# osudrl/cassie-mujoco-sim

Hardware: AMD Instinct MI355X
Metric: env-steps/sec (whole node) at N envs; max |qpos_err| vs CPU ref (higher is better)
Workload: dtype f64

## Files before the change

cassie-mujoco-sim_amd/csrc/env_step_collision.inc:

```
        constexpr int chain_rounds = [] {
            if constexpr (TOPO::is_static) { int r = 0, n = 1; while (n < DofLevels<TOPO>::depth() + 1) { n *= 4; ++r; } return r < 3 ? r : 3; }
            else return 3;
        }();
        int pf_jlim, pf_jtype, pf_jqadr, danc[9], blast, kvin;
        double pf_jmargin, pf_jlo, pf_jhi;
        auto request_behind_collision = [&](int lane_now) {
            const int pf_lj = lane_now < njnt ? lane_now : 0, pf_kd = lane_now < nv ? lane_now : 0, pf_bb = lane_now < nbody ? lane_now : 0;
            pf_jlim = m->jnt_limited[pf_lj]; pf_jtype = m->jnt_type[pf_lj]; pf_jqadr = m->jnt_qposadr[pf_lj];
            pf_jmargin = m->jnt_margin[pf_lj]; pf_jlo = m->jnt_range[pf_lj][0]; pf_jhi = m->jnt_range[pf_lj][1];
#pragma unroll
            for (int r = 0; r < 3 * chain_rounds; ++r) danc[r] = m->dof_anc4[pf_kd][r];
            blast = m->body_lastdof[pf_bb]; kvin = m->dof_vinsrc[pf_kd];
        };
        constexpr bool request_early = (FEAT & FEAT_HFIELD) == 0;
        if constexpr (request_early) request_behind_collision(lane);
        const int pair_bound = m->npair_simple;
        struct PairConst { int g1, g2, tt; double margin, rb1, rb2, s10, s11, s20, s21, s22; };
        auto request_pair = [&](int pp, PairConst &c) {
            const int ps = pp < pair_bound ? pp : 0;
            c.g1 = m->pair_geom1[ps]; c.g2 = m->pair_geom2[ps]; c.tt = m->pair_type[ps];
            c.margin = m->pair_margin[ps]; c.rb1 = m->pair_rbound[ps][0]; c.rb2 = m->pair_rbound[ps][1];
            c.s10 = m->pair_size[ps][0]; c.s11 = m->pair_size[ps][1];
            c.s20 = m->pair_size[ps][3]; c.s21 = m->pair_size[ps][4]; c.s22 = m->pair_size[ps][5];
        };
        PairConst pc;
        if constexpr (request_early) request_pair(lane, pc);
        int ncon = 0;
        int npass = m->npair_always;
        if (m->npair_simple > m->npair_always) {
            bool nearby = false;
            if (lane < m->ngeom && m->geom_farstatic[lane]) {
                const double rb = m->geom_rbound[lane] + m->geom_margin[lane];
                for (int ri = 0; ri < m->nroot; ++ri) {
                    const int r = m->root_body[ri];
                    double dv[3] = {S.x.s.geom_xpos[lane][0] - S.x.s.xpos[r][0], S.x.s.geom_xpos[lane][1] - S.x.s.xpos[r][1],
                                    S.x.s.geom_xpos[lane][2] - S.x.s.xpos[r][2]};
                    const double bound = PG->body_reach[r] + rb + 0.01;
                    if (dot3(dv, dv) < bound * bound) nearby = true;
                }
            }
            if (wv::ballot(nearby) != 0ull) npass = m->npair_simple;
        }
        CK_STAMP(21);
        constexpr int HF_REC = 1 + 10 * CM_HF_MAXC;
        static_assert(CM_MAXHFPAIR * HF_REC <= NB * 12 + NVP * 12, "the height-field result table must fit the cvel + cfrc + cdof_dot + buf tiles");
        static_assert(offsetof(decltype(S.x.s), buf) - offsetof(decltype(S.x.s), cvel) == sizeof(double) * (NB * 12 + NVP * 6), "those four tiles are contiguous");
        static_assert(CM_HF_PASS * CM_HF_SLOTS <= WV_WAVE && CM_HF_SLOTS_DENSE <= WV_WAVE, "a pass of the height-field pre-pass is one wave");
        double *const hfres = &S.x.s.cvel[0][0];
        const bool hf_on = (FEAT & FEAT_HFIELD) != 0 && env_hfield != nullptr && m->nhfpair > 0;
        const bool hf_prism = (FEAT & FEAT_HFIELD) != 0 && hf_on && (m->flags & CM_FLAG_HFPRISM) != 0;
        int ncon_prism = 0;
        if constexpr ((FEAT & FEAT_HFIELD) != 0) if (hf_prism) {
            static_assert(CM_MAXHFPAIR * HP_REC + 64 * 2 * CM_HP_MAXS / 8 <= NB * 12 + NVP * 12, "the per-pair records of the prism pass and its task table (a byte per task) fit the idle velocity tiles");
            CK_STAMP(44);
            ncon_prism = hfield_prism_wave(S, m, env_hfield, lane, hfres, MAXC);
            CK_STAMP(46);
        }
        if constexpr ((FEAT & FEAT_HFIELD) != 0) if (hf_on && !hf_prism) {
            const bool dense = (m->flags & CM_FLAG_HFDENSE) != 0;
            const int slots = dense ? CM_HF_SLOTS_DENSE : CM_HF_SLOTS, per_pass = dense ? WV_WAVE / CM_HF_SLOTS_DENSE : CM_HF_PASS;
            for (int h0 = 0; h0 < m->nhfpair; h0 += per_pass) {
                const int hl = dense ? lane / CM_HF_SLOTS_DENSE : lane / CM_HF_SLOTS;
                const int h = h0 + hl, k = lane - hl * slots;
                const bool act = hl < per_pass && h < m->nhfpair;
                const int p = m->hfpair[act ? h : 0];
                const int g1 = m->pair_geom1[p], g2 = m->pair_geom2[p], t2 = m->pair_type[p] >> 8;
                const double margin = m->pair_margin[p], s20 = m->pair_size[p][3], s21 = m->pair_size[p][4];
                const double *p1 = S.x.s.geom_xpos[g1], *m1 = S.x.s.geom_xmat[g1], *p2 = S.x.s.geom_xpos[g2], *m2 = S.x.s.geom_xmat[g2];
                const double axis[3] = {m2[2], m2[5], m2[8]};
                const double cell = 2 * m->hfield_size[0] / (m->hfield_ncol > 1 ? m->hfield_ncol - 1 : 1);
                int ni = 0;
                bool mine = act && k == 0;
                double t = 0;
                if (t2 == CM_GEOM_CAPSULE) {
                    ni = (int)ceil(2 * s21 / cell) - 1;
                    if (ni < 0) ni = 0;
                    if (ni > slots - 2) ni = slots - 2;
                    mine = act && k < 2 + ni;
                    t = k == 0 ? s21 : (k == 1 ? -s21 : s21 * (1.0 - 2.0 * (k - 1) / (ni + 1)));
                }
                RawContact rcs;
                rcs.dist = 1e300;
                bool has = false;
                {
                    double e[3] = {p2[0] + t * axis[0], p2[1] + t * axis[1], p2[2] + t * axis[2]};
                    static_assert(offsetof(SH_T, c_tran) + sizeof(S.c_tran) - offsetof(SH_T, c_dist) >= (size_t)HF_WORK_BYTES,
                                  "the contact tables hold the work area of hfield_spheres_wave");
                    CK_STAMP(44);
                    has = hfield_spheres_wave(rcs, m, env_hfield, p1, m1, mine, e, s20, margin, lane, &S.c_dist[0]) != 0;
                    CK_STAMP(45);
                }
                const int lead = lane - k;
                double dk[CM_HF_SLOTS_DENSE];
                const double mydist = has ? rcs.dist : 1e300;
#pragma unroll
                for (int q = 0; q < CM_HF_SLOTS_DENSE; ++q) {
                    if (q >= CM_HF_SLOTS && !dense) { dk[q] = 1e300; continue; }
                    const double v = wv::shfl(mydist, (lead + q) & 63);
                    dk[q] = q < slots ? v : 1e300;
                }
                int src0 = 0, src1 = 1;
                bool have0 = dk[0] < 1e299, have1 = dk[1] < 1e299;
                if (t2 == CM_GEOM_CAPSULE) {
                    int kmid = -1;
                    double dmid = 1e300;
#pragma unroll
                    for (int q = 2; q < CM_HF_SLOTS_DENSE; ++q) if (dk[q] < 1e299 && (kmid < 0 || dk[q] < dmid)) { kmid = q; dmid = dk[q]; }
                    if (kmid >= 0 && (!have0 || dmid < dk[0]) && (!have1 || dmid < dk[1])) {
                        const bool drop1 = !have0 ? false : (!have1 ? true : dk[0] <= dk[1]);
                        if (drop1) { src1 = kmid; have1 = true; } else { src0 = kmid; have0 = true; }
                    }
                } else {
                    have1 = false;
                }
                int nkeep = (have0 ? 1 : 0) + (have1 ? 1 : 0);
                double *rec = hfres + (size_t)(act ? h : 0) * HF_REC;
                int slot_of_me = (have0 && k == src0) ? 0 : ((have1 && k == src1) ? (have0 ? 1 : 0) : -1);
                if ((m->flags & CM_FLAG_HFMULTI) && t2 == CM_GEOM_CAPSULE) {
                    int rank = 0, cnt = 0;
#pragma unroll
                    for (int q = 0; q < CM_HF_SLOTS_DENSE; ++q) {
                        const bool valid = dk[q] < 1e299;
                        cnt += valid ? 1 : 0;
                        rank += (valid && (dk[q] < mydist || (dk[q] == mydist && q < k))) ? 1 : 0;
                    }
                    nkeep = cnt < CM_HF_MAXC ? cnt : CM_HF_MAXC;
                    slot_of_me = (has && rank < CM_HF_MAXC) ? rank : -1;
                }
                if (act && k == 0) rec[0] = (double)nkeep;
                if (act && slot_of_me >= 0) {
                    double *c = rec + 1 + 10 * slot_of_me;
                    c[0] = rcs.dist;
                    for (int i = 0; i < 3; ++i) { c[1 + i] = rcs.pos[i]; c[4 + i] = rcs.normal[i]; c[7 + i] = t2 == CM_GEOM_CAPSULE ? axis[i] : 0.0; }
                }
            }
            wv::sync();
            CK_STAMP(46);
        }
        if constexpr (!request_early) request_pair(lane, pc);
        if constexpr ((FEAT & FEAT_HFIELD) != 0) ncon = ncon_prism;
        for (int p0 = 0; p0 < npass; p0 += WV_WAVE) {
            const int p = p0 + lane;
            int n = 0;
            RawContact rc0, rc1;
            bool from_spread = false;
            int hfs = -1;
            if constexpr ((FEAT & FEAT_HFIELD) != 0) {
                const int slot = p < npass ? m->pair_hfslot[p] : -1;
                if (slot >= 0) {
                    from_spread = true;
                    if (hf_on && !hf_prism) {
                        const double *rec = hfres + (size_t)slot * HF_REC;
                        n = (int)rec[0];
                        hfs = slot;
                        rc0.dist = rec[1]; rc1.dist = rec[11];
                        for (int i = 0; i < 3; ++i) {
                            rc0.pos[i] = rec[2 + i]; rc0.normal[i] = rec[5 + i]; rc0.tangent[i] = rec[8 + i];
                            rc1.pos[i] = rec[12 + i]; rc1.normal[i] = rec[15 + i]; rc1.tangent[i] = rec[18 + i];
                        }
                    }
                }
            }
            if (p < npass && !from_spread) {
                const int g1 = pc.g1, g2 = pc.g2, tt = pc.tt;
                const int t1 = tt & 255, t2 = tt >> 8;
                const double margin = pc.margin;
                const double *p1 = S.x.s.geom_xpos[g1], *p2 = S.x.s.geom_xpos[g2];
                const double *m1 = S.x.s.geom_xmat[g1], *m2 = S.x.s.geom_xmat[g2];
                const double rb1 = pc.rb1, rb2 = pc.rb2;
                const double s10 = pc.s10, s11 = pc.s11, s20 = pc.s20, s21 = pc.s21, s22 = pc.s22;
                double dif[3] = {p2[0] - p1[0], p2[1] - p1[1], p2[2] - p1[2]};
                CK_STAMP(31);
                bool cull = false;
                if (rb1 > 0 && rb2 > 0) {
                    double bound = rb1 + rb2 + margin;
                    cull = dot3(dif, dif) > bound * bound;
                } else if (t1 == CM_GEOM_PLANE && rb2 > 0) {
                    double nn[3] = {m1[2], m1[5], m1[8]};
                    cull = dot3(dif, nn) > margin + rb2;
                }
                if (!cull) {
                    if (t1 == CM_GEOM_PLANE && t2 == CM_GEOM_SPHERE) {
                        n = plane_sphere(rc0, p1, m1, p2, s20, margin);
                    } else if (t1 == CM_GEOM_PLANE && t2 == CM_GEOM_CAPSULE) {
                        double axis[3] = {m2[2], m2[5], m2[8]};
                        RawContact tmp;
                        double e0[3] = {p2[0] + s21 * axis[0], p2[1] + s21 * axis[1], p2[2] + s21 * axis[2]};
                        if (plane_sphere(tmp, p1, m1, e0, s20, margin)) { rc0 = tmp; n = 1; }
                        double e1[3] = {p2[0] - s21 * axis[0], p2[1] - s21 * axis[1], p2[2] - s21 * axis[2]};
                        if (plane_sphere(tmp, p1, m1, e1, s20, margin)) { if (n == 0) rc0 = tmp; else rc1 = tmp; ++n; }
                        for (int i = 0; i < 3; ++i) { rc0.tangent[i] = axis[i]; rc1.tangent[i] = axis[i]; }
                    } else if (t1 == CM_GEOM_SPHERE && t2 == CM_GEOM_SPHERE) {
                        n = sphere_sphere(rc0, p1, s10, p2, s20, margin);
                    } else if (t1 == CM_GEOM_SPHERE && t2 == CM_GEOM_CAPSULE) {
                        double a2[3] = {m2[2], m2[5], m2[8]};
                        double d12[3] = {-dif[0], -dif[1], -dif[2]};
                        double x = clampd(dot3(a2, d12), -s21, s21);
                        double q2[3] = {p2[0] + a2[0] * x, p2[1] + a2[1] * x, p2[2] + a2[2] * x};
                        n = sphere_sphere(rc0, p1, s10, q2, s20, margin);
                    } else if (t1 == CM_GEOM_CAPSULE && t2 == CM_GEOM_CAPSULE) {
                        double a1[3] = {m1[2], m1[5], m1[8]}, a2[3] = {m2[2], m2[5], m2[8]};
                        double x1, x2;
                        segment_closest(p1, a1, s11, p2, a2, s21, x1, x2);
                        double q1[3] = {p1[0] + a1[0] * x1, p1[1] + a1[1] * x1, p1[2] + a1[2] * x1};
                        double q2[3] = {p2[0] + a2[0] * x2, p2[1] + a2[1] * x2, p2[2] + a2[2] * x2};
                        n = sphere_sphere(rc0, q1, s10, q2, s20, margin);
                    } else if (t1 == CM_GEOM_SPHERE && t2 == CM_GEOM_BOX) {
                        double sb[3] = {s20, s21, s22};
                        n = sphere_box(rc0, p1, s10, p2, m2, sb, margin);
                    } else if (t1 == CM_GEOM_CAPSULE && t2 == CM_GEOM_BOX) {
                        double sb[3] = {s20, s21, s22};
                        n = capsule_box(rc0, rc1, p1, m1, s10, s11, p2, m2, sb, margin);
                    } else {
                        warn |= WARN_UNSUPPORTED_PAIR;
                    }
                }
            }
            CK_STAMP(32);
            if (p0 + WV_WAVE < npass) request_pair(p + WV_WAVE, pc);
            const unsigned long long m1b = wv::ballot(n >= 1), m2b = wv::ballot(n >= 2);
            const unsigned long long below = (lane == 0) ? 0ull : (~0ull >> (64 - lane));
            int slot = ncon + wv::popc64(m1b & below) + wv::popc64(m2b & below);
            int more = 0;
            if constexpr ((FEAT & FEAT_HFIELD) != 0) {
                const unsigned long long m3b = wv::ballot(n >= 3), m4b = wv::ballot(n >= 4);
                slot += wv::popc64(m3b & below) + wv::popc64(m4b & below);
                more = wv::popc64(m3b) + wv::popc64(m4b);
                for (int extra = 2; extra < CM_HF_MAXC; ++extra)
                    if (n > extra && slot + extra < MAXC) {
                        const double *c = hfres + (size_t)hfs * HF_REC + 1 + 10 * extra;
                        RawContact rx;
                        rx.dist = c[0];
                        for (int i = 0; i < 3; ++i) { rx.pos[i] = c[1 + i]; rx.normal[i] = c[4 + i]; rx.tangent[i] = c[7 + i]; }
                        write_raw_contact(S, slot + extra, p, rx);
                    }
            }
            if (n >= 1 && slot < MAXC) write_raw_contact(S, slot, p, rc0);
            if (n >= 2 && slot + 1 < MAXC) write_raw_contact(S, slot + 1, p, rc1);
            ncon += wv::popc64(m1b) + wv::popc64(m2b) + more;
        }
        CK_STAMP(22);
        if constexpr (!request_early) request_behind_collision(lane);
        if constexpr ((FEAT & FEAT_WAVEPAIRS) != 0) for (int p = m->npair_simple; p < m->npair; ++p) {
            const int g1 = m->pair_geom1[p], g2 = m->pair_geom2[p], tt = m->pair_type[p];
            const int t1 = tt & 255, t2 = tt >> 8;
            const double margin = m->pair_margin[p];
            const double *p1 = S.x.s.geom_xpos[g1], *p2 = S.x.s.geom_xpos[g2];
            const double *m1 = S.x.s.geom_xmat[g1], *m2 = S.x.s.geom_xmat[g2];
            const double rb1 = m->pair_rbound[p][0], rb2 = m->pair_rbound[p][1];
            {
                double dif[3] = {p2[0] - p1[0], p2[1] - p1[1], p2[2] - p1[2]};
                bool cull = false;
                if (rb1 > 0 && rb2 > 0) { const double bound = rb1 + rb2 + margin; cull = dot3(dif, dif) > bound * bound; }
                else if (t1 == CM_GEOM_PLANE && rb2 > 0) { double nn[3] = {m1[2], m1[5], m1[8]}; cull = dot3(dif, nn) > margin + rb2; }
                if (cull) continue;
            }
            bool hit = false;
            int pairmax = 4;
            RawContact rc;
            if (t1 == CM_GEOM_PLANE && t2 == CM_GEOM_BOX) {
                if (lane < 8) {
                    const double sb0 = m->pair_size[p][3], sb1 = m->pair_size[p][4], sb2 = m->pair_size[p][5];
                    double nrm[3] = {m1[2], m1[5], m1[8]}, dif[3] = {p2[0] - p1[0], p2[1] - p1[1], p2[2] - p1[2]};
                    const double dist = dot3(dif, nrm);
                    double v[3] = {(lane & 1) ? sb0 : -sb0, (lane & 2) ? sb1 : -sb1, (lane & 4) ? sb2 : -sb2}, corner[3];
                    mulmatvec3(corner, m2, v);
                    const double ld = dot3(nrm, corner);
                    if (!(dist + ld > margin || ld > 0)) {
                        hit = true;
                        rc.dist = dist + ld;
                        for (int k = 0; k < 3; ++k) { rc.normal[k] = nrm[k]; rc.tangent[k] = 0; rc.pos[k] = corner[k] + p2[k] - nrm[k] * 0.5 * rc.dist; }
                    }
                }
            } else if (t1 == CM_GEOM_BOX && t2 == CM_GEOM_BOX) {
                double s1[3] = {m->pair_size[p][0], m->pair_size[p][1], m->pair_size[p][2]};
                double s2[3] = {m->pair_size[p][3], m->pair_size[p][4], m->pair_size[p][5]};
                pairmax = (m->flags & CM_FLAG_BOX8) ? 8 : 4;
                hit = box_box_lane(rc, lane, p1, m1, s1, p2, m2, s2, margin, pairmax);
            } else {
                warn |= WARN_UNSUPPORTED_PAIR;
            }
            const unsigned long long hb = wv::ballot(hit);
            const unsigned long long below = (lane == 0) ? 0ull : (~0ull >> (64 - lane));
            const int rank = wv::popc64(hb & below);
            if (hit && rank < pairmax && ncon + rank < MAXC) write_raw_contact(S, ncon + rank, p, rc);
            const int nh = wv::popc64(hb);
            ncon += nh < pairmax ? nh : pairmax;
        }
        const int ncon_found = ncon;
        if (ncon > capc) ncon = capc;
        wv::sync();
        finish_contacts(S, m, P, lane, ncon);
        unsigned long long lob, hib;
        {
            bool lo = false, hi = false;
            wv::keep(pf_jlim); wv::keep(pf_jtype);
            if (lane < njnt && pf_jlim && (pf_jtype == CM_JNT_HINGE || pf_jtype == CM_JNT_SLIDE)) {
                const double q = S.qpos[pf_jqadr];
                lo = q - pf_jlo < pf_jmargin;
                hi = pf_jhi - q < pf_jmargin;
            }
            lob = wv::ballot(lo); hib = wv::ballot(hi);
        }
        if constexpr (MAXR < WIDE_ROWS) {
            const bool may_go_down = io.down_rows > 0 && sub > sub_start;
            if (can_hand_over || may_go_down) {
                const int neq = m->neq;
                const bool eact = lane < neq && m->eq_active[lane < neq ? lane : 0] != 0;
                wv::sync();
                const int nfrictionless = wv::popc64(wv::ballot(lane < ncon && S.c_dim[lane < MAXC ? lane : 0] == 1));
                const int need = 3 * wv::popc64(wv::ballot(eact)) + wv::popc64(lob) + wv::popc64(hib) + 4 * ncon - 3 * nfrictionless;
                const bool up = can_hand_over && (need > capr || (ncon_found > capc && MAXC < m->maxcon));
                const bool down = !up && may_go_down && need <= io.down_rows;
                if (up || down) {
                    bailed = true; bailed_down = down;
                    if constexpr (NW == 2) { if (lane == 0) S.cmd[0] = 1; wv::publish(&S.cmd[4], sub + 1); }
                    break;
                }
            }
        }
        if (ncon_found > capc) warn |= WARN_CONTACT_FULL;
        if constexpr (NW == 1) if (io.drive_mode) {
            if (io.integrate) drive_level_io(io, S, m, env, lane, lastsub);
            wv::sync();
        }
        if constexpr (NW == 2) { CK_STAMP(33); wv::publish(&S.cmd[4], sub + 1); wv::wait_for(&S.cmd[3], sub + 1); }
        CK_STAMP(5);
```

cassie-mujoco-sim_amd/csrc/env_step_rows.inc:

```
        int r_ = lane;
        int rtype = -1, rid = 0, rsub = 0;
        int nefc = 0, nefc_before_contacts = 0;
        double rpos = 0, rmargin = 0, rR = 1.0, rK = 0, rB = 0, rimp = 1.0;
        const bool need_imu = lastsub || io.all_outputs_every_substep || (io.drive_mode && sub + 2 == nsub);
        const bool need_pos = lastsub || io.drive_mode || io.all_outputs_every_substep;
        const bool issens = lane < m->nsensor && need_pos;
        const int ls = issens ? lane : 0;
        SensorConsts sens_c;
        double ycol[NVP];
        double jvel = 0, jws = 0;
        const bool lastcol = !WIDE && lane == NROW - 1;
        for (int pass = 0; pass < (WIDE ? 2 : 1); ++pass) {
        if constexpr (WIDE) {
            if (pass == 1 && nefc <= NROW) break;
            r_ = NROW * pass + lane; rtype = -1; rid = 0; rsub = 0; nefc = 0; jvel = 0; jws = 0;
            rpos = 0; rmargin = 0; rR = 1.0; rK = 0; rB = 0; rimp = 1.0;
        }
        {
            const int neq = m->neq;
            const bool eact = lane < neq && m->eq_active[lane < neq ? lane : 0] != 0;
            const unsigned long long eall = neq >= 64 ? ~0ull : (1ull << neq) - 1;
            if (wv::ballot(eact) == eall && 3 * neq <= capr) {
                if (r_ < 3 * neq) { rtype = CM_CNSTR_EQUALITY; rid = r_ / 3; rsub = r_ - 3 * rid; }
                nefc = 3 * neq;
            } else
            for (int e = 0; e < neq; ++e) {
                if (!m->eq_active[e]) continue;
                if (nefc + 3 > capr) { warn |= WARN_CONSTRAINT_FULL; continue; }
                if (r_ >= nefc && r_ < nefc + 3) { rtype = CM_CNSTR_EQUALITY; rid = e; rsub = r_ - nefc; }
                nefc += 3;
            }
        }
        {
            for (unsigned long long any = lob | hib; any; any &= any - 1) {
                const int j = wv::popc64((any & (0ull - any)) - 1);
                for (int side = 0; side < 2; ++side) {
                    if (!(((side == 0 ? lob : hib) >> j) & 1ull)) continue;
                    if (nefc >= capr) { warn |= WARN_CONSTRAINT_FULL; continue; }
                    if (r_ == nefc) { rtype = CM_CNSTR_LIMIT_JOINT; rid = j; rsub = side; }
                    ++nefc;
                }
            }
        }
        nefc_before_contacts = nefc;
        const bool cpyr = lane < ncon && S.c_dim[lane < ncon ? lane : 0] == 3;
        if (wv::ballot(cpyr) == (ncon >= 64 ? ~0ull : (1ull << ncon) - 1) && nefc + 4 * ncon <= capr) {
            if (r_ >= nefc && r_ < nefc + 4 * ncon) { rtype = CM_CNSTR_CONTACT_PYRAMIDAL; rid = (r_ - nefc) >> 2; rsub = (r_ - nefc) & 3; }
            nefc += 4 * ncon;
        } else
        for (int c = 0; c < ncon; ++c) {
            const int dim = S.c_dim[c];
            if (dim != 1 && dim != 3) { warn |= WARN_UNSUPPORTED_PAIR; continue; }
            const int nrow = dim == 1 ? 1 : 2 * (dim - 1);
            if (nefc + nrow > capr) { warn |= WARN_CONSTRAINT_FULL; continue; }
            if (r_ >= nefc && r_ < nefc + nrow) {
                rtype = dim == 1 ? CM_CNSTR_CONTACT_FRICTIONLESS : CM_CNSTR_CONTACT_PYRAMIDAL;
                rid = c; rsub = r_ - nefc;
            }
            nefc += nrow;
        }

        CK_STAMP(25);
        double u3[3] = {0, 0, 0}, wp[3] = {0, 0, 0}, wm[3] = {0, 0, 0};
        unsigned long long maskp = 0, maskm = 0;
        int limdof = -1;
        double limsgn = 0, rdiag = 0, imp_pos = 0, rRscale = 1.0;
        double solref0 = 0.02, solref1 = 1, solimp[5] = {0.9, 0.95, 0.001, 0.5, 2};
        if (rtype == CM_CNSTR_EQUALITY) {
            if (rid != pf_eq) {
                pf_eb1 = m->eq_body1[rid]; pf_eb2 = m->eq_body2[rid]; pf_er1 = m->eq_root[rid][0]; pf_er2 = m->eq_root[rid][1];
            }
            maskp = m->eq_dofmask[rid][0]; maskm = m->eq_dofmask[rid][1];
            rdiag = P->eq_invweight[rid];
            solref0 = m->eq_solref[rid][0]; solref1 = m->eq_solref[rid][1];
            for (int i = 0; i < 5; ++i) solimp[i] = m->eq_solimp[rid][i];
            const int b1 = pf_eb1, b2 = pf_eb2;
            double l1[3] = {m->eq_data[rid][0], m->eq_data[rid][1], m->eq_data[rid][2]};
            double l2[3] = {m->eq_data[rid][3], m->eq_data[rid][4], m->eq_data[rid][5]};
            double a1[3], a2[3];
            mulmatvec3(a1, S.x.s.xmat[b1], l1);
            mulmatvec3(a2, S.x.s.xmat[b2], l2);
            for (int i = 0; i < 3; ++i) { a1[i] += S.x.s.xpos[b1][i]; a2[i] += S.x.s.xpos[b2][i]; }
            u3[0] = rsub == 0 ? 1.0 : 0.0; u3[1] = rsub == 1 ? 1.0 : 0.0; u3[2] = rsub == 2 ? 1.0 : 0.0;
            const double *c1 = S.com[pf_er1], *c2 = S.com[pf_er2];
            double o1[3] = {a1[0] - c1[0], a1[1] - c1[1], a1[2] - c1[2]};
            double o2[3] = {a2[0] - c2[0], a2[1] - c2[1], a2[2] - c2[2]};
            cross3(wp, o1, u3);
            cross3(wm, o2, u3);

            double res[3] = {a1[0] - a2[0], a1[1] - a2[1], a1[2] - a2[2]};
            rpos = rsub == 0 ? res[0] : (rsub == 1 ? res[1] : res[2]); rmargin = 0;
            imp_pos = sqrt(dot3(res, res));

        } else if (rtype == CM_CNSTR_LIMIT_JOINT) {
            const double q = S.qpos[m->jnt_qposadr[rid]];
            rpos = rsub == 0 ? q - m->jnt_range[rid][0] : m->jnt_range[rid][1] - q;
            rmargin = m->jnt_margin[rid];
            imp_pos = rpos;
            limdof = m->jnt_dofadr[rid];
            limsgn = rsub == 0 ? 1.0 : -1.0;
            rdiag = P->jnt_liminvweight[rid];
            solref0 = m->jnt_solref[rid][0]; solref1 = m->jnt_solref[rid][1];
            for (int i = 0; i < 5; ++i) solimp[i] = m->jnt_solimp[rid][i];
        } else if (rtype >= 0) {
            const int c = rid;
            const double *fr = S.c_frame[c];
            if (rtype == CM_CNSTR_CONTACT_PYRAMIDAL) {
                const int a = 1 + rsub / 2;
                const double mu = a <= 2 ? S.c_fri[c][0] : (a == 3 ? S.c_fri[c][1] : S.c_fri[c][2]);
                const double sg = (rsub & 1) ? -mu : mu;
                for (int i = 0; i < 3; ++i) u3[i] = fr[i] + sg * fr[3 * a + i];
                const double mu0 = S.c_fri[c][0];
                rRscale = 2 * mu0 * mu0;
            } else {
                for (int i = 0; i < 3; ++i) u3[i] = fr[i];
            }
            const double *c1 = S.com[S.c_root[c][0]], *c2 = S.com[S.c_root[c][1]];
            double o1[3] = {S.c_pos[c][0] - c1[0], S.c_pos[c][1] - c1[1], S.c_pos[c][2] - c1[2]};
            double o2[3] = {S.c_pos[c][0] - c2[0], S.c_pos[c][1] - c2[1], S.c_pos[c][2] - c2[2]};
            cross3(wp, o2, u3);
            cross3(wm, o1, u3);
            maskp = S.c_dofmask[c][1];
            maskm = S.c_dofmask[c][0];
            rpos = S.c_dist[c]; rmargin = S.c_margin[c]; imp_pos = rpos;
            const double tran = S.c_tran[c];
            const double mu_first = S.c_fri[c][0];
            rdiag = rtype == CM_CNSTR_CONTACT_PYRAMIDAL ? tran + mu_first * mu_first * tran : tran;
            solref0 = S.c_solref[c][0]; solref1 = S.c_solref[c][1];
            for (int i = 0; i < 5; ++i) solimp[i] = S.c_solimp[c][i];
        }
        CK_STAMP(26);
        if (rtype >= 0) {
            rimp = impedance(solimp, imp_pos, rmargin);
            rR = fmax(CM_MINVAL, (1 - rimp) * rdiag / rimp);
            if (rtype == CM_CNSTR_CONTACT_PYRAMIDAL) rR = fmax(CM_MINVAL, rRscale * rR);
            const double dmax = solimp[1];
            if (solref0 > 0) {
                double tc = solref0;
                if ((m->flags & CM_FLAG_REFSAFE) && tc < 2 * h) tc = 2 * h;
                rK = 1.0 / fmax(CM_MINVAL, dmax * dmax * tc * tc * solref1 * solref1);
                rB = 2.0 / fmax(CM_MINVAL, dmax * tc);
            } else {
                rK = -solref0 / fmax(CM_MINVAL, dmax * dmax);
                rB = -solref1 / fmax(CM_MINVAL, dmax);
            }
        }
        CK_STAMP(27);
        if constexpr (NW == 1) sens_c = request_sensor_consts(m, ls);
#pragma unroll
        for (int k0 = 0; k0 < NVP; k0 += 4) {
            double cc[4][6], qv[4], qw[4], qs[4];
#pragma unroll
            for (int kk = 0; kk < 4; ++kk) {
#pragma unroll
                for (int t = 0; t < 6; ++t) cc[kk][t] = S.cdof[k0 + kk][t];
                qv[kk] = S.qvel[k0 + kk]; qw[kk] = S.qacc_ws[k0 + kk];
                if constexpr (NW == 1) qs[kk] = S.qfrc_smooth[k0 + kk]; else qs[kk] = 0.0;
            }
            wv::sched_fence();
#pragma unroll
            for (int kk = 0; kk < 4; ++kk) {
                const int k = k0 + kk;
                double v = 0;
                if (TOPO::is_static ? k < TOPO::nv : k < nv) {
                    if (rtype >= 0) {
                        const double ul = u3[0] * cc[kk][3] + u3[1] * cc[kk][4] + u3[2] * cc[kk][5];
                        const double sp = bitf(maskp, k), sm = bitf(maskm, k);
                        v = sp * (ul + wp[0] * cc[kk][0] + wp[1] * cc[kk][1] + wp[2] * cc[kk][2]) -
                            sm * (ul + wm[0] * cc[kk][0] + wm[1] * cc[kk][1] + wm[2] * cc[kk][2]);
                        if (k == limdof) v = limsgn;
                        jvel += v * qv[kk];
                        jws += v * qw[kk];
                    } else if (lastcol) {
                        v = qs[kk];
                    }
                }
                ycol[k] = v;
            }
        }
        if constexpr (WIDE) {
            if (r_ < MAXR) {
#pragma unroll
                for (int k = 0; k < NVP; ++k) S.x.Yr[r_][k] = ycol[k];
                double *rt = S.x.rowt[r_];
                rt[0] = rR; rt[1] = rtype >= 0 ? -rB * jvel - rK * rimp * (rpos - rmargin) : 0.0; rt[2] = jws;
                rt[3] = rtype < 0 ? -1.0 : (rtype == CM_CNSTR_EQUALITY ? 0.0 : 1.0);
            }
            if (io.ext && pass == 0 && rtype == CM_CNSTR_EQUALITY && r_ < CM_MAXEQROW) {
                cm_ext_t *ex = io.ext + env;
                ex->eq_pos[r_] = rpos; ex->eq_id[r_] = rid;
#pragma unroll
                for (int k = 0; k < NVP; ++k) if (k < nv) ex->eq_J[r_][k] = ycol[k];
            }
        }
        }
        const int sb = NW == 1 ? sens_c.sb : 0;
        CK_STAMP(28);
        if constexpr (NW == 2) {
            if constexpr (WIDE) { if (lane == 0) S.x.turn[0] = nefc; }
            CK_STAMP(34); wv::block_barrier();
            if (lastcol) {
#pragma unroll
                for (int k = 0; k < NVP; ++k) ycol[k] = (TOPO::is_static ? k < TOPO::nv : k < nv) ? S.qfrc_smooth[k] : 0.0;
            }
        }
        const double raref = rtype >= 0 ? -rB * jvel - rK * rimp * (rpos - rmargin) : 0.0;

        int aslot = -1;
        if constexpr (NW == 1) aslot = sensors_before_solve(io, S, m, env, issens, ls, sens_c, need_imu, lastsub);
        CK_STAMP(29);
        if (io.xpos_out && isbody && lastsub) {
            for (int i = 0; i < 3; ++i) io.xpos_out[((size_t)env * io.sb + b) * 3 + i] = S.x.s.xpos[b][i];
            if (io.xquat_out) for (int i = 0; i < 4; ++i) io.xquat_out[((size_t)env * io.sb + b) * 4 + i] = S.x.s.xquat[b][i];
        }
        if (io.ext) {
            cm_ext_t *ex = io.ext + env;
            if (isbody) for (int i = 0; i < 6; ++i) ex->cvel[b][i] = S.x.s.cvel[b][i];
            if (isbody) for (int i = 0; i < 3; ++i) { ex->subtree_com[b][i] = S.com[broot > 0 ? broot : 0][i]; ex->xipos[b][i] = S.x.s.xipos[b][i]; }
            if (lane < m->nsite) {
                const int sb = m->site_bodyid[lane];
                double sp[3] = {m->site_pos[lane][0], m->site_pos[lane][1], m->site_pos[lane][2]};
                double sq[4] = {m->site_quat[lane][0], m->site_quat[lane][1], m->site_quat[lane][2], m->site_quat[lane][3]};
                double t[3], q[4], mm[9];
                mulmatvec3(t, S.x.s.xmat[sb], sp);
                for (int i = 0; i < 3; ++i) ex->site_xpos[lane][i] = t[i] + S.x.s.xpos[sb][i];
                mulquat(q, S.x.s.xquat[sb], sq);
                quat2mat(mm, q);
                for (int i = 0; i < 9; ++i) ex->site_xmat[lane][i] = mm[i];
            }
            if (isdof) for (int i = 0; i < 6; ++i) { ex->cdof[k_][i] = S.cdof[k_][i]; ex->cdof_dot[k_][i] = S.x.s.cdof_dot[k_][i]; }
            if (!WIDE && rtype == CM_CNSTR_EQUALITY && r_ < CM_MAXEQROW) {
                ex->eq_pos[r_] = rpos; ex->eq_id[r_] = rid;
#pragma unroll
                for (int k = 0; k < NVP; ++k) if (k < nv) ex->eq_J[r_][k] = ycol[k];
            }
            if (lane == 0) { int ne = 0; for (int e = 0; e < m->neq; ++e) if (m->eq_active[e] && ne + 3 <= capr) ne += 3; ex->ne = ne; }
            if (lane < ncon) {
                ex->con_geom1[lane] = m->geom_fullid[S.c_g1[lane]]; ex->con_geom2[lane] = m->geom_fullid[S.c_g2[lane]];
                ex->con_body1[lane] = m->geom_bodyid[S.c_g1[lane]]; ex->con_body2[lane] = m->geom_bodyid[S.c_g2[lane]];
                ex->con_dim[lane] = S.c_dim[lane]; ex->con_dist[lane] = S.c_dist[lane];
                for (int i = 0; i < 3; ++i) ex->con_pos[lane][i] = S.c_pos[lane][i];
                for (int i = 0; i < 9; ++i) ex->con_frame[lane][i] = S.c_frame[lane][i];
            }
        }
        int caddr = -1;
        const bool want_cfrc = io.body_cfrc && (sub == nsub - 1 || !io.integrate);
        if (io.ext || want_cfrc) {
            int acc = nefc_before_contacts;
            for (int c = 0; c < ncon; ++c) {
                const int dim = S.c_dim[c];
                if (dim != 1 && dim != 3) continue;
                const int nrow = dim == 1 ? 1 : 2 * (dim - 1);
                if (acc + nrow > capr) continue;
                if (c == lane) caddr = acc;
                acc += nrow;
            }
        }
        wv::sync();
        CK_STAMP(8);
```

cassie-mujoco-sim_amd/csrc/env_step_solve.inc:

```
        if constexpr (WIDE) {
            int iters = 0, nguarded = 0;
            const double f = wide_solve<NVP, TOPO>(S, m, P, 0, nefc, sub, iters, nguarded);
            CK_STAMP(11);

            static_assert(sizeof(S.c_solimp) >= (2 * NROW + 4) * sizeof(double), "the row forces are handed over through the contacts' solimp slots");
            double *const fbuf = &S.c_solimp[0][0];
            fbuf[lane] = f;
            if (lane == 0) { fbuf[2 * NROW] = (double)ncon; fbuf[2 * NROW + 1] = (double)nefc; fbuf[2 * NROW + 2] = (double)iters; fbuf[2 * NROW + 3] = (double)nguarded; }
            wv::block_barrier();
#ifdef CK_WIDE_PROFILE
            if (io.prof && lane < 12) io.prof[(size_t)env * NSTAMP + (lane < 6 ? 16 + lane : 22 + lane)] = (long long)S.x.stepv[lane / 6][lane % 6];
#endif
            if (io.ext || want_cfrc) {
                const int a0 = caddr >= 0 ? caddr : 0;
                double fn = 0, ft1 = 0, ft2 = 0;
                if (lane < ncon && caddr >= 0) {
                    const double f0 = fbuf[a0];
                    if (S.c_dim[lane] == 1) fn = f0;
                    else { const double f1 = fbuf[a0 + 1], f2 = fbuf[a0 + 2], f3 = fbuf[a0 + 3], mu = S.c_fri[lane][0]; fn = f0 + f1 + f2 + f3; ft1 = mu * (f0 - f1); ft2 = mu * (f2 - f3); }
                }
                if (io.ext) {
                    cm_ext_t *ex = io.ext + env;
                    if (lane < ncon) { ex->con_force[lane][0] = fn; ex->con_force[lane][1] = ft1; ex->con_force[lane][2] = ft2; }
                    if (lane == 0) { ex->ncon = ncon; ex->nefc = nefc; ex->solver_iter = iters; }
                }
                if (want_cfrc) {
                    if (lane < ncon) {
                        const double *fr = S.c_frame[lane];
                        double fw[3];
                        for (int j = 0; j < 3; ++j) fw[j] = fr[j] * fn + fr[3 + j] * ft1 + fr[6 + j] * ft2;
                        for (int j = 0; j < 3; ++j) S.c_pos[lane][j] = fw[j];
                    }
                    wv::sync();
                    if (isbody) {
                        double acc[3] = {0, 0, 0};
                        for (int c = 0; c < ncon; ++c) {
                            const int b1 = m->geom_bodyid[S.c_g1[c]], b2 = m->geom_bodyid[S.c_g2[c]];
                            const double sg = (b2 == b ? 1.0 : 0.0) - (b1 == b ? 1.0 : 0.0);
                            for (int j = 0; j < 3; ++j) acc[j] += sg * S.c_pos[c][j];
                        }
                        for (int j = 0; j < 3; ++j) io.body_cfrc[((size_t)env * io.sb + b) * 3 + j] = acc[j];
                    }
                    wv::sync();
                }
            }
            wv::block_barrier();
            CK_STAMP(37);
            if (wv::opaque(S.cmd[0])) { warn |= WARN_DIVERGED; break; }
            if (!io.integrate) break;
            time += h;
            continue;
        }
        if constexpr (TOPO::is_static) {
            double ta[NVP], tb[NVP], ra = 0, rb = 0;
            auto fetch = [&](int k, double (&t)[NVP], double &rs) {
#pragma unroll
                for (int i = k - 1; i >= 0; --i) if ((TOPO::table[k] >> i) & 1ull) t[i] = S.Lp[LPack<TOPO, NVP>::idx(k, i)];
                rs = S.rsd[k];
            };
            fetch(TOPO::nv - 1, ((TOPO::nv - 1) & 1) ? ta : tb, ((TOPO::nv - 1) & 1) ? ra : rb);
#pragma unroll
            for (int k = NVP - 1; k >= 0; --k) {
                if (k >= TOPO::nv) continue;
                if (k > 0) fetch(k - 1, ((k - 1) & 1) ? ta : tb, ((k - 1) & 1) ? ra : rb);
                wv::sched_fence();
                const double (&t)[NVP] = (k & 1) ? ta : tb;
                const double xk = ycol[k];
#pragma unroll
                for (int i = k - 1; i >= 0; --i) if ((TOPO::table[k] >> i) & 1ull) ycol[i] -= t[i] * xk;
                ycol[k] = xk * ((k & 1) ? ra : rb);
                wv::sched_fence();
            }
        } else {
#pragma unroll
            for (int k = NVP - 1; k >= 0; --k) {
                if (k >= nv) continue;
                const unsigned long long anc = m->dof_ancmask[k];
                const double xk = ycol[k];
#pragma unroll
                for (int i = k - 1; i >= 0; --i) {
                    if (!((anc >> i) & 1ull)) continue;
                    ycol[i] -= S.Lp[CK_TRI(k, i)] * xk;
                }
                ycol[k] = xk * S.rsd[k];
            }
        }
        if (r_ < MAXR || lastcol) {
            const int yrow = lastcol ? MAXR : r_;
#pragma unroll
            for (int k = 0; k < NVP; ++k) S.x.Yr[yrow][k] = ycol[k];
        }
        wv::sync();
        if constexpr (NW == 2) wv::publish(&S.cmd[2], sub + 1);
        CK_STAMP(9);

        double arow[MAXR];
        double diag_yy = 0;
        double rb = 0;
        constexpr bool gram_on_matrix_core = MAXR == 31 && NVP % 4 == 0;
        constexpr bool gram_in_place = MAXR == 47 && NVP == 40;
        if constexpr (gram_on_matrix_core) {
            constexpr int YP = EnvShared<NVP, LPack<TOPO, NVP>::count, MAXR>::YP;
            static_assert(2 * (MAXR + 1) * YP * sizeof(double) <= sizeof(S.x), "the Gram matrix is parked behind the staged tile");
            double (*Am)[YP] = (double (*)[YP])(&S.x.Yr[0][0] + (MAXR + 1) * YP);
            const int mi = lane & 15, mk = lane >> 4;
            double y0[NVP / 4], y1[NVP / 4];
#pragma unroll
            for (int kb = 0; kb < NVP / 4; ++kb) { y0[kb] = S.x.Yr[mi][4 * kb + mk]; y1[kb] = S.x.Yr[16 + mi][4 * kb + mk]; }
            wv::mfma_acc t00 = {{0, 0, 0, 0}}, t01 = {{0, 0, 0, 0}}, t11 = {{0, 0, 0, 0}};
#pragma unroll
            for (int kb = 0; kb < NVP / 4; ++kb) wv::mfma_f64_16x16x4_x3(y0[kb], y0[kb], t00, y0[kb], y1[kb], t01, y1[kb], y1[kb], t11);
            wv::mfma_f64_drain(t00, t01, t11);
#pragma unroll
            for (int v = 0; v < 4; ++v) {
                const int row = mk + 4 * v;
                Am[row][mi] = t00.c[v];
                Am[row][16 + mi] = t01.c[v];
                Am[16 + mi][row] = t01.c[v];
                Am[16 + row][16 + mi] = t11.c[v];
            }
            wv::sync();
            const int myrow = lane & 31;
#pragma unroll
            for (int t = 0; t < MAXR; ++t) arow[t] = Am[myrow][t];
            rb = Am[myrow][MAXR] - raref;
#pragma unroll
            for (int k = 0; k < NVP; ++k) wv::touch(ycol[k]);
            diag_yy = Am[myrow][myrow];
        } else if constexpr (gram_in_place) {
            constexpr int AP = 49, AR = MAXR + 1;
            static_assert(AR == 48, "three blocks of sixteen staged rows");
            static_assert(AR * AP * sizeof(double) <= sizeof(S.x), "the matrix fits the region of the staged tile");
            double (*Am)[AP] = (double (*)[AP])&S.x.Yr[0][0];
            const int mi = lane & 15, mk = lane >> 4;
            double y0[NVP / 4], y1[NVP / 4], y2[NVP / 4];
#pragma unroll
            for (int kb = 0; kb < NVP / 4; ++kb) { y0[kb] = S.x.Yr[mi][4 * kb + mk]; y1[kb] = S.x.Yr[16 + mi][4 * kb + mk]; y2[kb] = S.x.Yr[32 + mi][4 * kb + mk]; }
            wv::mfma_acc t00 = {{0, 0, 0, 0}}, t01 = {{0, 0, 0, 0}}, t11 = {{0, 0, 0, 0}}, t02 = {{0, 0, 0, 0}}, t12 = {{0, 0, 0, 0}}, t22 = {{0, 0, 0, 0}};
#pragma unroll
            for (int kb = 0; kb < NVP / 4; ++kb) wv::mfma_f64_16x16x4_x3(y0[kb], y2[kb], t02, y1[kb], y2[kb], t12, y2[kb], y2[kb], t22);
#pragma unroll
            for (int kb = 0; kb < NVP / 4; ++kb) wv::mfma_f64_16x16x4_x3(y0[kb], y0[kb], t00, y0[kb], y1[kb], t01, y1[kb], y1[kb], t11);
            wv::mfma_f64_drain(t00, t01, t11);
            wv::mfma_f64_drain(t02, t12, t22);
            wv::sync();
#pragma unroll
            for (int v = 0; v < 4; ++v) {
                const int row = mk + 4 * v;
                Am[row][mi] = t00.c[v];
                Am[row][16 + mi] = t01.c[v]; Am[16 + mi][row] = t01.c[v];
                Am[16 + row][16 + mi] = t11.c[v];
                Am[row][32 + mi] = t02.c[v]; Am[32 + mi][row] = t02.c[v];
                Am[16 + row][32 + mi] = t12.c[v]; Am[32 + mi][16 + row] = t12.c[v];
                Am[32 + row][32 + mi] = t22.c[v];
            }
            wv::sync();
            const int myrow = lane < AR ? lane : AR - 1;
            rb = Am[myrow][MAXR] - raref;
            diag_yy = Am[myrow][myrow];
#pragma unroll
            for (int t = 0; t < MAXR; ++t) arow[t] = Am[myrow][t];
            wv::sync();
            if (r_ < MAXR || lastcol) {
                const int yrow = lastcol ? MAXR : r_;
#pragma unroll
                for (int k = 0; k < NVP; ++k) S.x.Yr[yrow][k] = ycol[k];
            }
            wv::sync();
        }
        else if constexpr (NW == 2 && NVP > 32) {
#pragma unroll
            for (int r = 0; r < MAXR; ++r) {
                double acc = 0;
                if (r < nefc) {
#pragma unroll
                    for (int k0 = 0; k0 < NVP; k0 += NVP / 2) {
                        double ya[NVP / 2];
#pragma unroll
                        for (int k = 0; k < NVP / 2; ++k) ya[k] = S.x.Yr[r][k0 + k];
#pragma unroll
                        for (int k = 0; k < NVP / 2; ++k) acc = fma(ya[k], ycol[k0 + k], acc);
                    }
                }
                arow[r] = acc;
            }
            {
                double acc = 0;
#pragma unroll
                for (int k = 0; k < NVP; ++k) acc = fma(S.x.Yr[MAXR][k], ycol[k], acc);
                rb = acc - raref;
            }
        } else {
#pragma unroll
        for (int r = 0; r < MAXR; r += 2) {
            double acc0 = 0, acc1 = 0;
            if (r < nefc) {
                constexpr int YB1 = NVP > 32 ? NVP / 2 : NVP;
                double ya[NVP], yb[NVP];
#pragma unroll
                for (int k = 0; k < NVP; ++k) ya[k] = S.x.Yr[r][k];
#pragma unroll
                for (int k = 0; k < YB1; ++k) yb[k] = S.x.Yr[r + 1 < MAXR ? r + 1 : r][k];
                wv::sched_fence();
                if constexpr (NVP == 32) {
#pragma unroll
                    for (int k = 0; k < NVP; ++k) { acc0 = fma(ya[k], ycol[k], acc0); if (r + 1 < MAXR) acc1 = fma(yb[k], ycol[k], acc1); }
                } else if constexpr (NVP == 40) {
#pragma unroll
                    for (int k = 0; k < YB1; ++k) { acc0 = fma(ya[k], ycol[k], acc0); if (r + 1 < MAXR) acc1 = fma(yb[k], ycol[k], acc1); }
                    wv::sched_fence();
#pragma unroll
                    for (int k = YB1; k < NVP; ++k) yb[k] = S.x.Yr[r + 1 < MAXR ? r + 1 : r][k];
#pragma unroll
                    for (int k = YB1; k < NVP; ++k) { acc0 = fma(ya[k], ycol[k], acc0); if (r + 1 < MAXR) acc1 = fma(yb[k], ycol[k], acc1); }
                } else {
                double a0 = 0, a1 = 0, a2 = 0, a3 = 0;
#pragma unroll
                for (int k = 0; k < NVP; k += 4) {
                    a0 += ya[k] * ycol[k]; a1 += ya[k + 1] * ycol[k + 1];
                    a2 += ya[k + 2] * ycol[k + 2]; a3 += ya[k + 3] * ycol[k + 3];
                }
                acc0 = (a0 + a1) + (a2 + a3);
                if constexpr (YB1 < NVP) {
                    wv::sched_fence();
#pragma unroll
                    for (int k = YB1; k < NVP; ++k) yb[k] = S.x.Yr[r + 1 < MAXR ? r + 1 : r][k];
                }
                if (r + 1 < MAXR) {
                    double b0 = 0, b1 = 0, b2 = 0, b3 = 0;
#pragma unroll
                    for (int k = 0; k < NVP; k += 4) {
                        b0 += yb[k] * ycol[k]; b1 += yb[k + 1] * ycol[k + 1];
                        b2 += yb[k + 2] * ycol[k + 2]; b3 += yb[k + 3] * ycol[k + 3];
                    }
                    acc1 = (b0 + b1) + (b2 + b3);
                }
                }
            }
            arow[r] = acc0;
            if (r + 1 < MAXR) arow[r + 1] = acc1;
        }
        {
            double acc = 0;
#pragma unroll
            for (int k = 0; k < NVP; ++k) acc = fma(S.x.Yr[MAXR][k], ycol[k], acc);
            rb = acc - raref;
        }
        }
        CK_STAMP(10);

        const bool isrow = rtype >= 0;
        const bool clampf = isrow && rtype != CM_CNSTR_EQUALITY;
        double Aii = 1.0;
        if constexpr (gram_on_matrix_core || gram_in_place) { if (isrow) Aii = diag_yy + rR; }
        else if (isrow) {
            if constexpr (NVP == 32 || NVP == 40) {
                double d = 0;
#pragma unroll
                for (int k = 0; k < NVP; ++k) d = fma(ycol[k], ycol[k], d);
                Aii = d + rR;
            } else {
                double d0 = 0, d1 = 0, d2 = 0, d3 = 0;
#pragma unroll
                for (int k = 0; k < NVP; k += 4) {
                    d0 += ycol[k] * ycol[k]; d1 += ycol[k + 1] * ycol[k + 1];
                    d2 += ycol[k + 2] * ycol[k + 2]; d3 += ycol[k + 3] * ycol[k + 3];
                }
                Aii = ((d0 + d1) + (d2 + d3)) + rR;
            }
        }
        const double invAii = 1.0 / Aii;
        double f = 0, res = isrow ? rb : 0.0;
        int iters = 0, nguarded = 0;
        if (nefc > 0) {
            if (m->flags & CM_FLAG_WARMSTART) {
                if (isrow) {
                    f = -(jws - raref) / rR;
                    if (clampf && f < 0) f = 0;
                }
                double af0 = 0, af1 = 0, af2 = 0, af3 = 0;
#pragma unroll
                for (int t = 0; t < MAXR; t += 4) {
                    if (t < nefc) {
                        af0 += arow[t] * wv::readlane(f, t);
                        if (t + 1 < MAXR) af1 += arow[t + 1] * wv::readlane(f, t + 1);
                        if (t + 2 < MAXR) af2 += arow[t + 2] * wv::readlane(f, t + 2);
                        if (t + 3 < MAXR) af3 += arow[t + 3] * wv::readlane(f, t + 3);
                    }
                }
                const double af = ((af0 + af1) + (af2 + af3)) + (isrow ? rR * f : 0.0);
                double cost = wv::wave_sum(isrow ? f * (rb + 0.5 * af) : 0.0);
                if (cost > 0) f = 0;
                else if (isrow) res = rb + af;
            }
        CK_STAMP(30);
            const double scale = 1.0 / (P->meaninertia * (nv > 1 ? nv : 1));
            const double halfAii = 0.5 * Aii;
            const double flo = clampf ? 0.0 : -1e300;
            const double ninvAii = -invAii;
            double sres = res * ninvAii;
#pragma unroll
            for (int t = 0; t < MAXR; ++t) arow[t] *= ninvAii;
            const double cdiag = isrow ? rR * ninvAii : 0.0;
            const int maxiter = m->iterations;
            const double tolerance = m->tolerance;
            const bool shortcut_ok = 0.5 * tolerance > (double)MAXR * 1e-10 * scale;
            if constexpr (NW == 2 && CK_PRIO_W0_PGS != CK_PRIO_W0) wv::set_priority<CK_PRIO_W0_PGS>();
            while (iters < maxiter) {
                const int nrows = wv::opaque(nefc);
                bool converged;
                {
                    const double f0 = f, s0 = sres;
                    double mys = 0;
                    const double lo_f = flo - f;
                    pgs_rows_fast<0, MAXR>(arow, nrows, r_, lo_f, sres, mys);
                    const double mydelta = wv::max_raw(mys, lo_f);
                    const double change = (r_ < nrows) ? mydelta * (halfAii * mydelta - Aii * mys) : 0.0;
                    const float tol = (float)tolerance;
                    const bool one_row_decides = shortcut_ok && wv::ballot(-(float)change * (float)scale > 2.5f * tol) != 0ull;
                    const float est = one_row_decides ? 4.0f * tol : -wv::wave_sum_f32((float)change) * (float)scale;
                    if (wv::ballot(change > 1e-10) != 0ull || wv::debug_force_guarded()) {
                        double improvement = 0;
                        f = f0; sres = s0; ++nguarded;
                        pgs_rows<0, MAXR>(arow, nrows, r_, Aii, halfAii, flo, f, sres, improvement);
                        sres = fma(cdiag, f - f0, sres);
                        converged = improvement * scale < tolerance;
                    } else {
                        if (r_ < nrows) { f += mydelta; sres = fma(cdiag, mydelta, sres); }
                        if (est < 0.5f * tol) converged = true;
                        else if (est > 2.0f * tol) converged = false;
                        else {
                            const double tree = -wv::wave_sum(change) * scale, tolv = tolerance;
                            if (fabs(tree - tolv) > 1e-9 * tolv) converged = tree < tolv;
                            else
                            {
                                double improvement = 0;
                                for (int t = 0; t < nrows; ++t) improvement -= wv::readlane(change, t);
                                converged = improvement * scale < tolerance;
                            }
                        }
                    }
                }
                ++iters;
                if (converged) break;
            }
        }
        if constexpr (NW == 2 && CK_PRIO_W0_PGS != CK_PRIO_W0) wv::set_priority<CK_PRIO_W0>();
        CK_STAMP(11);
        if (io.ext || want_cfrc) {
            const int a0 = caddr >= 0 ? caddr : 0;
            const double f0 = wv::shfl(f, a0), f1 = wv::shfl(f, (a0 + 1) & 63), f2 = wv::shfl(f, (a0 + 2) & 63), f3 = wv::shfl(f, (a0 + 3) & 63);
            double fn = 0, ft1 = 0, ft2 = 0;
            if (lane < ncon && caddr >= 0) {
                if (S.c_dim[lane] == 1) fn = f0;
                else { const double mu = S.c_fri[lane][0]; fn = f0 + f1 + f2 + f3; ft1 = mu * (f0 - f1); ft2 = mu * (f2 - f3); }
            }
            if (io.ext) {
                cm_ext_t *ex = io.ext + env;
                if (lane < ncon) { ex->con_force[lane][0] = fn; ex->con_force[lane][1] = ft1; ex->con_force[lane][2] = ft2; }
                if (lane == 0) { ex->ncon = ncon; ex->nefc = nefc; ex->solver_iter = iters; }
            }
            if (want_cfrc) {
                if (lane < ncon) {
                    const double *fr = S.c_frame[lane];
                    double fw[3];
                    for (int j = 0; j < 3; ++j) fw[j] = fr[j] * fn + fr[3 + j] * ft1 + fr[6 + j] * ft2;
                    for (int j = 0; j < 3; ++j) S.c_pos[lane][j] = fw[j];
                }
                wv::sync();
                if (isbody) {
                    double acc[3] = {0, 0, 0};
                    for (int c = 0; c < ncon; ++c) {
                        const int b1 = m->geom_bodyid[S.c_g1[c]], b2 = m->geom_bodyid[S.c_g2[c]];
                        const double sg = (b2 == b ? 1.0 : 0.0) - (b1 == b ? 1.0 : 0.0);
                        for (int j = 0; j < 3; ++j) acc[j] += sg * S.c_pos[c][j];
                    }
                    for (int j = 0; j < 3; ++j) io.body_cfrc[((size_t)env * io.sb + b) * 3 + j] = acc[j];
                }
                wv::sync();
            }
        }

        if constexpr (NW == 2) {
            static_assert(sizeof(S.c_solimp) >= 68 * sizeof(double), "the row forces are handed over through the contacts' solimp slots");
            double *const fbuf = &S.c_solimp[0][0];
            fbuf[lane] = f;
            if (lane == 0) { fbuf[64] = (double)ncon; fbuf[65] = (double)nefc; fbuf[66] = (double)iters; fbuf[67] = (double)nguarded; }
            wv::block_barrier();
            wv::block_barrier();
            CK_STAMP(37);
            if (wv::opaque(S.cmd[0])) { warn |= WARN_DIVERGED; break; }
            if (!io.integrate) break;
            time += h;
            continue;
        }
        const int pf_u = lane < nu ? lane : 0, pf_ej = lane < njnt ? lane : 0;
        const double pf_agear = m->act_gear[pf_u], pf_kdamp = P->dof_damping[isdof ? k_ : 0];
        const int pf_adof = m->act_dofid[pf_u], pf_ejt = m->jnt_type[pf_ej], pf_eqa = m->jnt_qposadr[pf_ej], pf_eda = m->jnt_dofadr[pf_ej];
        double qacc;
        {
            double z = isdof ? S.x.Yr[MAXR][k_] : 0.0;
            {
                double z1 = 0, z2 = 0, z3 = 0;
                const int kk = isdof ? k_ : 0;
                int r = 0;
                for (; r + 4 <= nefc; r += 4) {
                    const double y0 = S.x.Yr[r][kk], y1 = S.x.Yr[r + 1][kk], y2 = S.x.Yr[r + 2][kk], y3 = S.x.Yr[r + 3][kk];
                    z += y0 * wv::readlane(f, r); z1 += y1 * wv::readlane(f, r + 1);
                    z2 += y2 * wv::readlane(f, r + 2); z3 += y3 * wv::readlane(f, r + 3);
                }
                for (; r < nefc; ++r) z += S.x.Yr[r][kk] * wv::readlane(f, r);
                z = (z + z1) + (z2 + z3);
                if (!isdof) z = 0.0;
            }
            if (isdof) z *= S.rsd[k_];
            double lrow[NVP];
            stage_factor_row<NVP, TOPO>(S, k_, isdof, lrow);
            qacc = solve_forward<NVP, TOPO>(z, lrow, lane, nv);
        }
        {
            const bool badv = isdof && (!(qacc == qacc) || fabs(qacc) > 1e10);
            if (wv::ballot(badv) != 0ull) { warn |= WARN_DIVERGED; break; }
        }
        if (isdof) S.qacc[k_] = qacc;
        wv::sync();
        CK_STAMP(12);

        outputs_after_qacc(io, S, m, env, lane, isdof, k_, nu, qacc, aslot, sb, need_imu, lastsub, pf_agear * S.qvel[pf_adof], ncon, nefc, iters, nguarded);
        if (!io.integrate) break;
        CK_STAMP(13);

        {
            double lcol[NVP], lrowh[NVP];
            stage_factor_h<NVP, TOPO>(S, k_, isdof, nv, lcol, lrowh);
            const double dih = isdof ? S.dinvH[k_] : 0.0;
            euler_step<NVP, TOPO>(S, m, lane, isdof, k_, nv, njnt, h, qacc, lcol, lrowh, dih, pf_kdamp, pf_ejt, pf_eqa, pf_eda);
        }
        time += h;
        CK_STAMP(14);
    }
```

cassie-mujoco-sim_amd/csrc/env_step_wave1.inc:

```
    if constexpr (NW == 2) {
        if (wid == 1) {
            for (int sub1 = sub_start;;) {
                const int pb = isbody ? b : 0;
                const double mass = P->body_mass[pb];
                double iner[3], imat[9];
                for (int i = 0; i < 3; ++i) iner[i] = P->body_inertia[pb][i];
                for (int i = 0; i < 9; ++i) imat[i] = m->body_imat[pb][i];
                CK_STAMP(35);
                wv::block_barrier();
                if (wv::opaque(S.cmd[0])) return -1;
                wv::set_priority<(FEAT & FEAT_HFIELD) != 0 ? CK_PRIO_W1_FJ_HFIELD : CK_PRIO_W1_FJ>();
                CK_STAMP(36);
                double ximat[9] = {1, 0, 0, 0, 1, 0, 0, 0, 1};
                if (isbody && b > 0) {
                    double xm[9];
                    for (int i = 0; i < 9; ++i) xm[i] = S.x.s.xmat[b][i];
                    for (int i = 0; i < 3; ++i)
                        for (int c = 0; c < 3; ++c) ximat[3 * i + c] = xm[3 * i] * imat[c] + xm[3 * i + 1] * imat[3 + c] + xm[3 * i + 2] * imat[6 + c];
                }
                double col[NVP], colh[NVP];
                mass_matrix_columns<NVP, TOPO, FEAT, NW>(io, S, m, env, ids, mass, iner, ximat, col, colh);
                wv::publish(&S.cmd[3], sub1 + 1);
                CK_STAMP(38);
                factor_pair_by_height<NVP, TOPO, 0>(m, P, h, S, col, colh, lane);
                constexpr bool park_colh = NVP > 32;
                if constexpr (park_colh) {
                    if (isdof) {
#pragma unroll
                        for (int i = 0; i < NVP; ++i) {
                            if (i >= TOPO::nv) continue;
                            if (i == k_) S.dinvH[k_] = colh[i];
                            else if (i > k_ && LP::col_has(i, k_)) S.LHp[LP::col_idx(i, k_)] = colh[i];
                        }
                    }
                    wv::sync();
                }
                wv::wait_for(&S.cmd[4], sub1 + 1);
                if (wv::opaque(S.cmd[0])) return -1;
                if (io.drive_mode) {
                    if (io.integrate) drive_level_io(io, S, m, env, lane, sub1 == nsub - 1);
                    wv::sync();
                }
                CK_STAMP(4);
                {
                    const int kd = isdof ? k_ : 0;
                    const double kdamp = P->dof_damping[kd], kstiff = PS->dof_stiffness[kd], kref = PS->dof_springref[kd];
                    const double kgear = m->dof_gear[kd], klo = m->dof_ctrl_lo[kd], khi = m->dof_ctrl_hi[kd];
                    const int kq = m->dof_qadr[kd], ka = m->dof_act[kd];
                    wv::wait_for(&S.cmd[1], sub1 + 1);
                    bias_forces_and_qfrc_smooth<NVP, (NVP > 32)>(io, S, m, env, ids, kdamp, kstiff, kref, kgear, klo, khi, kq, ka);
                }
                const bool lastsub1 = sub1 == nsub - 1 || !io.integrate;
                const bool need_imu1 = lastsub1 || io.all_outputs_every_substep || (io.drive_mode && sub1 + 2 == nsub);
                const bool issens1 = lane < m->nsensor && (lastsub1 || io.drive_mode || io.all_outputs_every_substep);
                const int ls1 = issens1 ? lane : 0;
                const SensorConsts sens_c1 = request_sensor_consts(m, ls1);
                const int aslot1 = sensors_before_solve(io, S, m, env, issens1, ls1, sens_c1, need_imu1, lastsub1);
                CK_STAMP(47);
                wv::block_barrier();
                wv::set_priority<CK_PRIO_W1_JP>();
                CK_STAMP(39);
                if constexpr (WIDE) {
                    int it1 = 0, ng1 = 0;
                    const double f1 = wide_solve<NVP, TOPO>(S, m, P, 1, wv::opaque(S.x.turn[0]), sub1, it1, ng1);
                    (&S.c_solimp[0][0])[NROW + lane] = f1;
                }
                if constexpr (park_colh) {
#pragma unroll
                    for (int i = 0; i < NVP; ++i) {
                        double v = 0.0;
                        if (i < TOPO::nv && isdof) {
                            if (i == k_) v = S.dinvH[k_];
                            else if (i > k_ && LP::col_has(i, k_)) v = S.LHp[LP::col_idx(i, k_)];
                        }
                        colh[i] = v;
                    }
                    wv::sync();
                }
                factor_pair_by_height<NVP, TOPO, 1>(m, P, h, S, col, colh, lane);
                {
                    const bool lastsub = lastsub1, need_imu = need_imu1;
                    const int sb = sens_c1.sb, aslot = aslot1;
                    const int pf_u = lane < nu ? lane : 0, pf_ej = lane < njnt ? lane : 0;
                    const double pf_agear = m->act_gear[pf_u], pf_kdamp = P->dof_damping[isdof ? k_ : 0];
                    const int pf_adof = m->act_dofid[pf_u], pf_ejt = m->jnt_type[pf_ej], pf_eqa = m->jnt_qposadr[pf_ej], pf_eda = m->jnt_dofadr[pf_ej];
                    const double *const fbuf = &S.c_solimp[0][0];
                    double lrow[NVP];
                    constexpr bool stage_h_early = NVP <= 32;
                    if constexpr (stage_h_early) stage_factor_row<NVP, TOPO>(S, k_, isdof, lrow);
                    double lcol[NVP], lrowh[NVP];
                    if constexpr (stage_h_early) stage_factor_h<NVP, TOPO, 0>(S, k_, isdof, nv, lcol, lrowh);
                    const double rsdk = isdof ? S.rsd[k_] : 0.0;
                    const int kk = isdof ? k_ : 0;
                    constexpr bool stage_y = MAXR <= 31;
                    double ycolk[stage_y ? MAXR + 1 : 1];
                    if constexpr (stage_y) {
                        wv::wait_for(&S.cmd[2], sub1 + 1);
#pragma unroll
                        for (int r = 0; r <= MAXR; ++r) ycolk[r] = S.x.Yr[r][kk];
                    }
                    wv::block_barrier();
                    wv::set_priority<CK_PRIO_W1_PE>();
                    const double f = fbuf[lane], f_hi = WIDE ? fbuf[NROW + lane] : 0.0;
                    constexpr int FB = WIDE ? 2 * NROW : NROW;
                    const int ncon = (int)fbuf[FB], nefc = (int)fbuf[FB + 1], iters = (int)fbuf[FB + 2], nguarded = (int)fbuf[FB + 3];
                    double z, z1 = 0, z2 = 0, z3 = 0;
                    if constexpr (stage_y) {
                        z = isdof ? ycolk[MAXR] : 0.0;
#pragma unroll
                        for (int r = 0; r < MAXR; r += 4) {
                            if (r + 4 <= nefc) {
                                z += ycolk[r] * wv::readlane(f, r); z1 += ycolk[r + 1 < MAXR ? r + 1 : r] * wv::readlane(f, r + 1);
                                z2 += ycolk[r + 2 < MAXR ? r + 2 : r] * wv::readlane(f, r + 2); z3 += ycolk[r + 3 < MAXR ? r + 3 : r] * wv::readlane(f, r + 3);
                            } else {
#pragma unroll
                                for (int j = 0; j < 4; ++j) if (r + j < nefc && r + j < MAXR) z += ycolk[r + j < MAXR ? r + j : r] * wv::readlane(f, r + j);
                            }
                        }
                    } else {
                        z = isdof ? S.x.Yr[MAXR][k_] : 0.0;
                        auto frow = [&](int r) { if constexpr (WIDE) return r < NROW ? wv::readlane(f, r) : wv::readlane(f_hi, r - NROW); else return wv::readlane(f, r); };
                        int r = 0;
                        for (; r + 4 <= nefc; r += 4) {
                            const double y0 = S.x.Yr[r][kk], y1 = S.x.Yr[r + 1][kk], y2 = S.x.Yr[r + 2][kk], y3 = S.x.Yr[r + 3][kk];
                            z += y0 * frow(r); z1 += y1 * frow(r + 1);
                            z2 += y2 * frow(r + 2); z3 += y3 * frow(r + 3);
                        }
                        for (; r < nefc; ++r) z += S.x.Yr[r][kk] * frow(r);
                    }
                    z = (z + z1) + (z2 + z3);
                    if (!isdof) z = 0.0;
                    if (isdof) z *= rsdk;
                    if constexpr (stage_h_early) stage_factor_h<NVP, TOPO, 1>(S, k_, isdof, nv, lcol, lrowh);
                    const double dih = isdof ? S.dinvH[k_] : 0.0;
                    if constexpr (!stage_h_early) stage_factor_row<NVP, TOPO>(S, k_, isdof, lrow);
                    wv::sched_fence();
                    const double qacc = solve_forward<NVP, TOPO>(z, lrow, lane, nv);
                    {
                        const bool badv = isdof && (!(qacc == qacc) || fabs(qacc) > 1e10);
                        if (wv::ballot(badv) != 0ull) {
                            if (lane == 0) S.cmd[0] = 2;
                            wv::block_barrier();
                            return -1;
                        }
                    }
                    if (isdof) S.qacc[k_] = qacc;
                    const double av = pf_agear * S.qvel[pf_adof];
                    wv::sync();
                    CK_STAMP(12);
                    if (io.integrate) {
                        if constexpr (!stage_h_early) stage_factor_h<NVP, TOPO>(S, k_, isdof, nv, lcol, lrowh);
                        euler_step<NVP, TOPO>(S, m, lane, isdof, k_, nv, njnt, h, qacc, lcol, lrowh, dih, pf_kdamp, pf_ejt, pf_eqa, pf_eda);
                    }
                    CK_STAMP(13);
                    wv::block_barrier();
                    wv::set_priority<CK_PRIO_W1_EF>();
                    outputs_after_qacc(io, S, m, env, lane, isdof, k_, nu, qacc, aslot, sb, need_imu, lastsub, av, ncon, nefc, iters, nguarded);
                    CK_STAMP(14);
                }
                if (!io.integrate || ++sub1 >= nsub) return -1;
            }
        }
    }
```

cassie-mujoco-sim_amd/csrc/physics_kernel.h:

```cpp
#ifndef CASSIE_PHYSICS_KERNEL_H
#define CASSIE_PHYSICS_KERNEL_H

#include <wave.h>

#include "cm_model.h"
#include "topo_static.h"

#include "pk_types.h"
#include "pk_math.h"
#include "pk_safety.h"
#include "pk_collision.h"
#include "pk_factor_solve.h"
#include "pk_stages.h"
#include "pk_wide_solve.h"

namespace ck {


constexpr int ENV_STEP_WENT_DOWN = 1 << 20;

template <int NVP, class TOPO, int FEAT, int MAXR, int NW>
WV_DEVICE int env_step(const PhysIO &io, EnvShared<NVP, LPack<TOPO, NVP>::count, MAXR> &S, int env, int sub_start, int nsub) {
    typedef LPack<TOPO, NVP> LP;
    static_assert(NW == 1 || NW == 2, "one or two wavefronts per env");
    static_assert(NW == 1 || TOPO::is_static, "the two-wave form exists for the compile-time topologies");
    const int wid = NW == 2 ? wv::wave_id() : 0;
    if constexpr (NW == 2) { if (wid == 0) wv::set_priority<CK_PRIO_W0>(); }
    constexpr int prio_kin = (FEAT & FEAT_HFIELD) != 0 ? CK_PRIO_W0 : CK_PRIO_W0_KIN;

    static_assert(LP::covers() && LP::distinct(), "packed factor rows must hold every ancestor pair, each in its own slot");
    typedef EnvShared<NVP, LPack<TOPO, NVP>::count, MAXR> SH_T;
    constexpr int MAXC = SH_T::MAXC;
    constexpr bool WIDE = SH_T::WIDE;
    static_assert(!WIDE || (NW == 2 && MAXR == WIDE_ROWS), "the 127-row instantiation spreads its solve over the two wavefronts of an env");
    const ModelPtr m_launch = (ModelPtr)(io.models + (size_t)env * io.model_stride);
    ModelPtr m = m_launch;
    const ParamPtr P = io.envparams ? (ParamPtr)(io.envparams + (size_t)env) : (ParamPtr)&m_launch->params;
    const ParamPtr PG = m_launch->env_geom ? P : (ParamPtr)&m_launch->params, PS = m_launch->env_springs ? P : (ParamPtr)&m_launch->params;
    int lane = wv::lane();
    const int nq = m->nq, nv = m->nv, nu = m->nu, nbody = m->nbody, njnt = m->njnt;
    const int capr = m->maxefc < MAXR ? m->maxefc : MAXR, capc = m->maxcon < MAXC ? m->maxcon : MAXC;
    const bool can_hand_over = MAXR < WIDE_ROWS && io.has_next != 0 && io.progress != nullptr && (MAXR < m->maxefc || MAXC < m->maxcon);
    const double h = m->timestep;
    int warn = 0;

    if (NW == 1 || wid == 0) {
    if (lane == 0) { S.cmd[0] = 0; S.cmd[1] = 0; S.cmd[2] = 0; S.cmd[3] = 0; S.cmd[4] = 0; }
    if constexpr (WIDE) { if (lane == 0) { S.x.turn[0] = 0; S.x.turn[1] = 0; S.x.turn[2] = 0; S.x.turn[3] = 0; } }
    if (lane < nq) S.qpos[lane] = io.qpos[(size_t)env * io.sq + lane];
    if (lane < nv) {
        S.qvel[lane] = io.qvel[(size_t)env * io.sqv + lane];
        S.qacc_ws[lane] = io.qacc_warmstart[(size_t)env * io.sv + lane];
    }
    if (lane < nu) S.ctrl[lane] = io.ctrl[(size_t)env * io.su + lane];
    if (lane < NB && !wv::test_skip_com_init()) { S.com[lane][0] = 0.0; S.com[lane][1] = 0.0; S.com[lane][2] = 0.0; }
    if (io.drive_mode) {
        if (lane < m->nsensordata) S.sens[lane] = io.sensordata[(size_t)env * io.ssd + lane];
        if (lane < nu) S.actvel[lane] = io.actuator_velocity[(size_t)env * io.su + lane];
        drive_state_load(io, S, env, lane);
        drive_consts_load(io, S, m, env, lane);
    }
    }
    double time = io.time[env];

    int b = lane;
    bool isbody = b < nbody;
    const int depth = isbody ? m->body_depth[b] : -1;
    const int bparent = isbody ? m->body_parentid[b] : 0;
    const int broot = isbody ? m->body_rootid[b] : -1;
    const int bjn = isbody ? m->body_jntnum[b] : 0;
    const int bj0 = (isbody && bjn > 0) ? m->body_jntadr[b] : 0;
    const int bend = isbody ? m->body_subtreeend[b] : 0;
    const unsigned long long bdofmask = isbody ? m->body_dofmask[b] : 0ull;
    const int bjt = (isbody && bjn > 0) ? m->jnt_type[bj0] : -1;
    const int bjq = (isbody && bjn > 0) ? m->jnt_qposadr[bj0] : 0;
    int k_ = lane;
    bool isdof = k_ < nv;
    const int kjnt = isdof ? m->dof_jntid[k_] : 0;
    const int kbody = isdof ? m->dof_bodyid[k_] : 0;
    const int kjt = isdof ? m->jnt_type[kjnt] : -1;
    const int kda = isdof ? m->jnt_dofadr[kjnt] : 0;
    const int kqa = isdof ? m->jnt_qposadr[kjnt] : 0;
    const int kroot = isdof ? m->body_rootid[kbody] : 0;
    const int kbend = isdof ? m->body_subtreeend[kbody] : 0;
    const unsigned long long kdesc = isdof ? m->dof_descmask[k_] : 0ull;
    const unsigned long long kvelmask = isdof ? m->dof_velmask[k_] : 0ull;
    int kact = -1;
    for (int u = 0; u < nu; ++u) if (isdof && m->act_dofid[u] == k_) kact = u;
    const LaneIds ids = {nbody, nv, broot, bend, kjnt, kbody, kjt, kda, kroot, kbend, kdesc};
    wv::sync();

#include "env_step_wave1.inc"

    const float *env_hfield = nullptr;
    if constexpr ((FEAT & FEAT_HFIELD) != 0) {
        bool clamped;
        env_hfield = terrain_grid(io.hfield, io.hfield_stride, io.hfield_index, io.hfield_nterrain, env, &clamped);
        if (clamped && lane == 0 && wid == 0) wv::atomic_or(io.warn + env, WARN_TERRAIN_INDEX);
    }

    bool bailed = false, bailed_down = false;
    int sub = sub_start;
    for (; sub < nsub; ++sub) {
        const bool lastsub = sub == nsub - 1 || !io.integrate;
        const bool need_quat = lastsub || io.ext != nullptr || io.all_outputs_every_substep || (io.drive_mode && sub + 2 == nsub);
        {
            bool badv = false;
            if (lane < nq) { double v = S.qpos[lane]; badv |= !(v == v) || fabs(v) > 1e10; }
            if (lane < nv) { double v = S.qvel[lane]; badv |= !(v == v) || fabs(v) > 1e10; }
            if (wv::ballot(badv) != 0ull) {
                warn |= WARN_DIVERGED;
                if constexpr (NW == 2) { if (lane == 0) S.cmd[0] = 1; wv::block_barrier(); }
                break;
            }
        }
        if (io.drive_mode) {
        } else if (io.pd_ptarget) {
            if (lane < nu) {
                const size_t o = (size_t)env * io.su + lane;
                const double ratio = m->act_gear[lane], tmax = m->act_ctrlrange[lane][1];
                const double q = S.qpos[m->act_qposadr[lane]], qd = S.qvel[m->act_dofid[lane]];
                const double tau = io.pd_kp[o] * (io.pd_ptarget[o] - q) - io.pd_kd[o] * qd;
                const double wmax = m->act_maxrpm[lane] * (2.0 * 3.14159265358979323846 / 60.0);
                const double tlim = clampd(2 * tmax * (1 - fabs(ratio * qd) / wmax), 0.0, tmax);
                S.ctrl[lane] = copysign(fmin(fabs(tau / ratio), tlim), tau);
            }
            wv::sync();
        }
        CK_STAMP(0);
        if constexpr (NW == 2 && prio_kin != CK_PRIO_W0) wv::set_priority<prio_kin>();

        double Rl[9] = {1, 0, 0, 0, 1, 0, 0, 0, 1}, pl[3] = {0, 0, 0}, qlq[4] = {1, 0, 0, 0};
        constexpr int kin_rounds = [] {
            if constexpr (TOPO::is_static) { int r = 0, n = 1; while (n < TOPO::body_levels) { n *= 3; ++r; } return r < 1 ? 1 : r; }
            else return 3;
        }();
        int kanc[2 * kin_rounds];
#pragma unroll
        for (int r = 0; r < 2 * kin_rounds; ++r) kanc[r] = isbody ? m->body_anc3[b][r] : 0;
        const bool isfree = bjt == CM_JNT_FREE;
        if constexpr (TOPO::is_static) {
            {
                const auto *kr = &m->body_kin[isbody ? b : 0];
                const int nsl = kr->nslide, j0 = kr->jnt0, jr = kr->rot_jnt, jt = kr->rot_type, qa = kr->rot_qadr;
                int sqa[CM_MAXSLIDE];
                double sref[CM_MAXSLIDE], sax[CM_MAXSLIDE][3], spo[CM_MAXSLIDE][3];
#pragma unroll
                for (int sl = 0; sl < CM_MAXSLIDE; ++sl) {
                    sqa[sl] = kr->slide_qadr[sl]; sref[sl] = kr->slide_ref[sl];
                    for (int i = 0; i < 3; ++i) { sax[sl][i] = kr->slide_axis_p[sl][i]; spo[sl][i] = kr->slide_pos_p[sl][i]; }
                }
                const double jref = kr->rot_ref;
                double jp[3], ja[3], jpp[3], xl[3], q0[4];
                for (int i = 0; i < 3; ++i) { jp[i] = kr->rot_pos[i]; ja[i] = kr->rot_axis[i]; jpp[i] = kr->rot_pos_p[i]; xl[i] = kr->rot_axis_p[i]; }
                for (int i = 0; i < 9; ++i) Rl[i] = kr->mat[i];
                for (int i = 0; i < 3; ++i) pl[i] = kr->pos[i];
                for (int i = 0; i < 4; ++i) q0[i] = kr->quat[i];
#pragma unroll
                for (int sl = 0; sl < CM_MAXSLIDE; ++sl) {
                    const double d = S.qpos[sqa[sl]] - sref[sl];
                    if (sl < nsl) for (int i = 0; i < 3; ++i) { S.x.s.xanchor[j0 + sl][i] = pl[i] + spo[sl][i]; S.x.s.xaxis[j0 + sl][i] = sax[sl][i]; }
                    for (int i = 0; i < 3; ++i) pl[i] += sax[sl][i] * d;
                }
                for (int i = 0; i < 4; ++i) qlq[i] = q0[i];
                double sn, cs;
                sincos_bounded(jt == CM_JNT_HINGE ? 0.5 * (S.qpos[qa] - jref) : 0.0, sn, cs);
                if (jr >= 0) {
                    double qj[4];
                    if (jt == CM_JNT_HINGE) {
                        qj[0] = cs; qj[1] = ja[0] * sn; qj[2] = ja[1] * sn; qj[3] = ja[2] * sn;
                    } else {
                        const int qo = jt == CM_JNT_FREE ? qa + 3 : qa;
                        for (int i = 0; i < 4; ++i) qj[i] = S.qpos[qo + i];
                        normalize4_fast(qj);
                        if (jt == CM_JNT_FREE) for (int i = 0; i < 3; ++i) pl[i] = S.qpos[qa + i];
                    }
                    double al[3], Rq[9], Rn[9], r[3];
                    for (int i = 0; i < 3; ++i) { al[i] = pl[i] + jpp[i]; S.x.s.xanchor[jr][i] = al[i]; S.x.s.xaxis[jr][i] = xl[i]; }
                    quat2mat(Rq, qj);
                    for (int i = 0; i < 3; ++i)
                        for (int c = 0; c < 3; ++c) Rn[3 * i + c] = Rl[3 * i] * Rq[c] + Rl[3 * i + 1] * Rq[3 + c] + Rl[3 * i + 2] * Rq[6 + c];
                    for (int i = 0; i < 9; ++i) Rl[i] = Rn[i];
                    if (need_quat) mulquat(qlq, q0, qj);
                    mulmatvec3(r, Rl, jp);
                    for (int i = 0; i < 3; ++i) pl[i] = al[i] - r[i];
                }
            }
        } else
        if (isbody && b > 0) {
            double bpos[3], bq[4];
            for (int i = 0; i < 3; ++i) bpos[i] = m->body_pos[b][i];
            for (int i = 0; i < 4; ++i) bq[i] = m->body_quat[b][i];
            if (isfree) {
                for (int i = 0; i < 3; ++i) pl[i] = S.qpos[bjq + i];
                for (int i = 0; i < 4; ++i) qlq[i] = S.qpos[bjq + 3 + i];
                normalize4(qlq);
                quat2mat(Rl, qlq);
                for (int i = 0; i < 3; ++i) { S.x.s.xanchor[bj0][i] = pl[i]; S.x.s.xaxis[bj0][i] = (i == 2) ? 1.0 : 0.0; }
            } else {
                for (int i = 0; i < 9; ++i) Rl[i] = m->body_mat[b][i];
                for (int i = 0; i < 3; ++i) pl[i] = bpos[i];
                for (int i = 0; i < 4; ++i) qlq[i] = bq[i];
                int jt_n = 0, qa_n = 0;
                double jp_n[3] = {0, 0, 0}, ja_n[3] = {0, 0, 0}, ref_n = 0;
                if (bjn > 0) {
                    jt_n = m->jnt_type[bj0]; qa_n = m->jnt_qposadr[bj0]; ref_n = m->jnt_ref[bj0];
                    for (int i = 0; i < 3; ++i) { jp_n[i] = m->jnt_pos[bj0][i]; ja_n[i] = m->jnt_axis[bj0][i]; }
                }
                for (int jj = 0; jj < bjn; ++jj) {
                    const int j = bj0 + jj, jt = jt_n, qa = qa_n;
                    const double jref = ref_n;
                    double jp[3] = {jp_n[0], jp_n[1], jp_n[2]}, ja[3] = {ja_n[0], ja_n[1], ja_n[2]};
                    if (jj + 1 < bjn) {
                        jt_n = m->jnt_type[j + 1]; qa_n = m->jnt_qposadr[j + 1]; ref_n = m->jnt_ref[j + 1];
                        for (int i = 0; i < 3; ++i) { jp_n[i] = m->jnt_pos[j + 1][i]; ja_n[i] = m->jnt_axis[j + 1][i]; }
                    }
                    double al[3], xl[3];
                    mulmatvec3(al, Rl, jp);
                    for (int i = 0; i < 3; ++i) al[i] += pl[i];
                    mulmatvec3(xl, Rl, ja);
                    for (int i = 0; i < 3; ++i) { S.x.s.xanchor[j][i] = al[i]; S.x.s.xaxis[j][i] = xl[i]; }
                    if (jt == CM_JNT_SLIDE) {
                        const double sl = S.qpos[qa] - jref;
                        for (int i = 0; i < 3; ++i) pl[i] += xl[i] * sl;
                    } else {
                        double qj[4];
                        if (jt == CM_JNT_BALL) { for (int i = 0; i < 4; ++i) qj[i] = S.qpos[qa + i]; normalize4(qj); }
                        else {
                            const double ang = S.qpos[qa] - jref;
                            const double sn = sin(0.5 * ang);
                            qj[0] = cos(0.5 * ang); qj[1] = ja[0] * sn; qj[2] = ja[1] * sn; qj[3] = ja[2] * sn;
                        }
                        double Rq[9], Rn[9], r[3];
                        quat2mat(Rq, qj);
                        for (int i = 0; i < 3; ++i)
                            for (int c = 0; c < 3; ++c) Rn[3 * i + c] = Rl[3 * i] * Rq[c] + Rl[3 * i + 1] * Rq[3 + c] + Rl[3 * i + 2] * Rq[6 + c];
                        for (int i = 0; i < 9; ++i) Rl[i] = Rn[i];
                        if (need_quat) mulquat(qlq, qlq, qj);
                        mulmatvec3(r, Rl, jp);
                        for (int i = 0; i < 3; ++i) pl[i] = al[i] - r[i];
                    }
                }
            }
        }
        CK_STAMP(16);
        const int pf_b = isbody ? b : 0, pf_g = lane < m->ngeom ? lane : -1, pf_gs = pf_g >= 0 ? pf_g : 0;
        const int pf_jpb = lane < njnt ? m->jnt_parentbody[lane] : -1, pf_gb = m->geom_bodyid[pf_gs];
        const double pf_mass = P->body_mass[pf_b];
        double pf_ipos[3], pf_imat[9], pf_iner[3], pf_gpos[3], pf_gmat[9];
        for (int i = 0; i < 3; ++i) { pf_ipos[i] = P->body_ipos[pf_b][i]; pf_iner[i] = P->body_inertia[pf_b][i]; pf_gpos[i] = PG->geom_pos[pf_gs][i]; }
        for (int i = 0; i < 9; ++i) { pf_imat[i] = m->body_imat[pf_b][i]; pf_gmat[i] = PG->geom_mat[pf_gs][i]; }
        double xm[9], xp[3], xq[4];
        for (int i = 0; i < 9; ++i) xm[i] = Rl[i];
        for (int i = 0; i < 3; ++i) xp[i] = pl[i];
        for (int i = 0; i < 4; ++i) xq[i] = qlq[i];
        {
            double *bufB = &S.x.s.cinert[0][0];
            auto park = [&](bool in_pose_tiles) {
                if (lane < NB) {
                    if (in_pose_tiles) {
                        for (int i = 0; i < 9; ++i) S.x.s.xmat[lane][i] = xm[i];
                        for (int i = 0; i < 3; ++i) S.x.s.xpos[lane][i] = xp[i];
                        if (need_quat) for (int i = 0; i < 4; ++i) S.x.s.xquat[lane][i] = xq[i];
                    } else {
                        for (int i = 0; i < 9; ++i) bufB[lane * 17 + i] = xm[i];
                        for (int i = 0; i < 3; ++i) bufB[lane * 17 + 9 + i] = xp[i];
                        if (need_quat) for (int i = 0; i < 4; ++i) bufB[lane * 17 + 12 + i] = xq[i];
                    }
                }
                wv::sync();
            };
            auto compose = [&](const double *Ra, const double *pa, const double *qa) {
                double Rn[9], pn[3];
                for (int i = 0; i < 3; ++i) {
                    for (int c = 0; c < 3; ++c) Rn[3 * i + c] = Ra[3 * i] * xm[c] + Ra[3 * i + 1] * xm[3 + c] + Ra[3 * i + 2] * xm[6 + c];
                    pn[i] = pa[i] + (Ra[3 * i] * xp[0] + Ra[3 * i + 1] * xp[1] + Ra[3 * i + 2] * xp[2]);
                }
                for (int i = 0; i < 9; ++i) xm[i] = Rn[i];
                for (int i = 0; i < 3; ++i) xp[i] = pn[i];
                if (need_quat) mulquat(xq, qa, xq);
            };
            constexpr bool first_in_pose_tiles = (kin_rounds & 1) == 0;
            park(first_in_pose_tiles);
#pragma unroll
            for (int r = 0; r < kin_rounds; ++r) {
                const bool from_pose_tiles = first_in_pose_tiles == ((r & 1) == 0);
                const int a1 = kanc[2 * r], a2 = kanc[2 * r + 1];
                double R1[9], p1[3], q1[4] = {1, 0, 0, 0}, R2[9], p2[3], q2[4] = {1, 0, 0, 0};
                if (from_pose_tiles) {
                    for (int i = 0; i < 9; ++i) { R1[i] = S.x.s.xmat[a1][i]; R2[i] = S.x.s.xmat[a2][i]; }
                    for (int i = 0; i < 3; ++i) { p1[i] = S.x.s.xpos[a1][i]; p2[i] = S.x.s.xpos[a2][i]; }
                    if (need_quat) for (int i = 0; i < 4; ++i) { q1[i] = S.x.s.xquat[a1][i]; q2[i] = S.x.s.xquat[a2][i]; }
                } else {
                    for (int i = 0; i < 9; ++i) { R1[i] = bufB[a1 * 17 + i]; R2[i] = bufB[a2 * 17 + i]; }
                    for (int i = 0; i < 3; ++i) { p1[i] = bufB[a1 * 17 + 9 + i]; p2[i] = bufB[a2 * 17 + 9 + i]; }
                    if (need_quat) for (int i = 0; i < 4; ++i) { q1[i] = bufB[a1 * 17 + 12 + i]; q2[i] = bufB[a2 * 17 + 12 + i]; }
                }
                if (a1 > 0) compose(R1, p1, q1);
                if (a2 > 0) compose(R2, p2, q2);
                park(!from_pose_tiles);
            }
        }
        if (b == 0) for (int i = 0; i < 3; ++i) S.x.s.xipos[0][i] = 0;
        double ximat[9] = {1, 0, 0, 0, 1, 0, 0, 0, 1};
        if (isbody && b > 0) {
            double xi[3];
            const double *ip = pf_ipos, *im = pf_imat;
            mulmatvec3(xi, xm, ip);
            for (int i = 0; i < 3; ++i) S.x.s.xipos[b][i] = xp[i] + xi[i];
            for (int i = 0; i < 3; ++i)
                for (int c = 0; c < 3; ++c) ximat[3 * i + c] = xm[3 * i] * im[c] + xm[3 * i + 1] * im[3 + c] + xm[3 * i + 2] * im[6 + c];
        }
        const int jpb = pf_jpb;
        if (jpb >= 0) {
            const int pb = jpb;
            double al[3] = {S.x.s.xanchor[lane][0], S.x.s.xanchor[lane][1], S.x.s.xanchor[lane][2]};
            double xl[3] = {S.x.s.xaxis[lane][0], S.x.s.xaxis[lane][1], S.x.s.xaxis[lane][2]}, aw[3], xw[3];
            mulmatvec3(aw, S.x.s.xmat[pb], al);
            mulmatvec3(xw, S.x.s.xmat[pb], xl);
            for (int i = 0; i < 3; ++i) { S.x.s.xanchor[lane][i] = aw[i] + S.x.s.xpos[pb][i]; S.x.s.xaxis[lane][i] = xw[i]; }
        }
        if constexpr (NW == 2) wv::block_barrier();
        if constexpr (NW == 2 && prio_kin != CK_PRIO_W0) wv::set_priority<CK_PRIO_W0>();
        CK_STAMP(1);

        if (pf_g >= 0) {
            const int g = pf_g, gb = pf_gb;
            const double *gp = pf_gpos, *gm = pf_gmat;
            double t[3];
            const double *R = S.x.s.xmat[gb];
            mulmatvec3(t, R, gp);
            for (int i = 0; i < 3; ++i) S.x.s.geom_xpos[g][i] = t[i] + S.x.s.xpos[gb][i];
            for (int i = 0; i < 3; ++i)
                for (int c = 0; c < 3; ++c) S.x.s.geom_xmat[g][3 * i + c] = R[3 * i] * gm[c] + R[3 * i + 1] * gm[3 + c] + R[3 * i + 2] * gm[6 + c];
        }
        if constexpr (NW == 2) wv::sync();

        CK_STAMP(17);
        double col[NVP], colh[NVP];
        if constexpr (NW == 1) mass_matrix_columns<NVP, TOPO, FEAT, NW>(io, S, m, env, ids, pf_mass, pf_iner, ximat, col, colh);

        constexpr bool by_height = TOPO::is_static;
        if constexpr (NW == 2) {
        } else if constexpr (by_height) {
            factor_pair_by_height<NVP, TOPO>(m, P, h, S, col, colh, lane);
        } else {
            factor_pair_in_registers<NVP, TOPO>(m, P, h, col, colh, lane, nv, S.dinv, S.rsd, S.dinvH);
            if (isdof) {
#pragma unroll
                for (int k = 1; k < NVP; ++k) {
                    if (TOPO::is_static ? k >= TOPO::nv : k >= nv) continue;
                    if (k > k_) { S.Lp[CK_TRI(k, k_)] = col[k]; S.LHp[CK_TRI(k, k_)] = colh[k]; }
                }
            }
        }
        if constexpr (NW == 1) CK_STAMP(4);

#include "env_step_collision.inc"

        double mycvel[6], mycacc[6];
#pragma unroll
        for (int r = 0; r < 3 * chain_rounds; ++r) { wv::keep(danc[r]); if (!isdof) danc[r] = -1; }
        wv::keep(blast); wv::keep(kvin);
        if (!isbody) blast = -1;
        if (!isdof) kvin = -1;
        const int kd = isdof ? k_ : 0;
        const double kdamp = P->dof_damping[kd], kstiff = PS->dof_stiffness[kd], kref = PS->dof_springref[kd];
        const double kgear = m->dof_gear[kd], klo = m->dof_ctrl_lo[kd], khi = m->dof_ctrl_hi[kd];
        const int kq = m->dof_qadr[kd], ka = m->dof_act[kd];
        auto chain_sums = [&](double (&acc)[6]) {
            if (lane < NVP) for (int t = 0; t < 6; ++t) S.x.s.buf[lane][t] = acc[t];
            wv::sync();
#pragma unroll
            for (int r = 0; r < chain_rounds; ++r) {
                double up[3][6];
#pragma unroll
                for (int i = 0; i < 3; ++i) {
                    const int a = danc[3 * r + i] >= 0 ? danc[3 * r + i] : 0;
                    for (int t = 0; t < 6; ++t) up[i][t] = S.x.s.buf[a][t];
                }
                wv::sync();
#pragma unroll
                for (int i = 0; i < 3; ++i)
                    if (danc[3 * r + i] >= 0) for (int t = 0; t < 6; ++t) acc[t] += up[i][t];
                if (lane < NVP) for (int t = 0; t < 6; ++t) S.x.s.buf[lane][t] = acc[t];
                wv::sync();
            }
        };
        {
            double term[6];
            const double qd = isdof ? S.qvel[lane < NVP ? lane : 0] : 0.0;
            for (int t = 0; t < 6; ++t) term[t] = (lane < NVP ? S.cdof[lane < NVP ? lane : 0][t] : 0.0) * qd;
            chain_sums(term);
            for (int t = 0; t < 6; ++t) mycvel[t] = blast >= 0 ? S.x.s.buf[blast >= 0 ? blast : 0][t] : 0.0;
            double vin[6];
            for (int t = 0; t < 6; ++t) vin[t] = kvin >= 0 ? S.x.s.buf[kvin >= 0 ? kvin : 0][t] : 0.0;
            if (lane < NB) for (int t = 0; t < 6; ++t) S.x.s.cvel[lane][t] = mycvel[t];
            if (lane < NVP) {
                double cdd[6] = {0, 0, 0, 0, 0, 0}, cd[6];
                for (int i = 0; i < 6; ++i) cd[i] = S.cdof[lane][i];
                if (isdof && !(kjt == CM_JNT_FREE && k_ - kda < 3)) cross_motion(cdd, vin, cd);
                for (int i = 0; i < 6; ++i) S.x.s.cdof_dot[lane][i] = cdd[i];
                for (int t = 0; t < 6; ++t) term[t] = cdd[t] * qd;
            } else {
                for (int t = 0; t < 6; ++t) term[t] = 0;
            }
            wv::sync();
            CK_STAMP(23);
            chain_sums(term);
            for (int t = 0; t < 6; ++t) mycacc[t] = blast >= 0 ? S.x.s.buf[blast >= 0 ? blast : 0][t] : 0.0;
            mycacc[3] -= m->gravity[0]; mycacc[4] -= m->gravity[1]; mycacc[5] -= m->gravity[2];
            wv::sync();
            if (lane < NB) for (int t = 0; t < 6; ++t) S.x.s.buf[lane][t] = mycacc[t];
            wv::sync();
        }
        if (lane < NB) {
            double f6[6] = {0, 0, 0, 0, 0, 0};
            if (isbody && b > 0) {
                double t1[6], t2[6], t3[6], ci[10];
                for (int i = 0; i < 10; ++i) ci[i] = S.x.s.cinert[b][i];
                mul_inert_vec(t1, ci, mycacc);
                mul_inert_vec(t2, ci, mycvel);
                cross_force(t3, mycvel, t2);
                for (int i = 0; i < 6; ++i) f6[i] = t1[i] + t3[i];
            }
            for (int i = 0; i < 6; ++i) S.x.s.cfrc[lane][i] = f6[i];
        }
        wv::sync();
        CK_STAMP(24);
        if constexpr (NW == 2) {
            wv::publish(&S.cmd[1], sub + 1);
        } else bias_forces_and_qfrc_smooth<NVP>(io, S, m, env, ids, kdamp, kstiff, kref, kgear, klo, khi, kq, ka);
        const int pf_eq = lane < 3 * m->neq ? lane / 3 : 0;
        int pf_eb1 = m->eq_body1[pf_eq], pf_eb2 = m->eq_body2[pf_eq], pf_er1 = m->eq_root[pf_eq][0], pf_er2 = m->eq_root[pf_eq][1];

#include "env_step_rows.inc"

#include "env_step_solve.inc"

    if (io.progress && lane == 0 && (!io.resume || bailed)) {
        io.progress[env] = bailed ? sub : nsub;
        if (bailed && !bailed_down && io.handover_out_list) io.handover_out_list[io.env0 + wv::atomic_add(io.handover_out_count, 1)] = env;
    }
    if (io.integrate && io.drive_mode) {
        drive_state_store(io, S, env, lane);
        if (lane < nu) io.ctrl[(size_t)env * io.su + lane] = S.ctrl[lane];
        if (bailed) {
            if (lane < m->nsensordata) io.sensordata[(size_t)env * io.ssd + lane] = S.sens[lane];
            if (lane < nu) io.actuator_velocity[(size_t)env * io.su + lane] = S.actvel[lane];
            if (lane < CM_NUM_DRIVES) {
                double *meas = io.meas + (size_t)env * CM_MEAS_DIM;
                meas[CM_MEAS_DRIVE_POS + lane] = S.drv_pos[lane]; meas[CM_MEAS_DRIVE_VEL + lane] = S.drv_vel[lane];
            }
        }
    }
    if (io.integrate) {
        if (lane < nq) io.qpos[(size_t)env * io.sq + lane] = S.qpos[lane];
        if (lane < nv) {
            io.qvel[(size_t)env * io.sqv + lane] = S.qvel[lane];
            io.qacc_warmstart[(size_t)env * io.sv + lane] = S.qacc_ws[lane];
        }
        if (lane == 0) io.time[env] = time;
    }
    {
        int w = 0;
        for (int bit = 1; bit <= 8; bit <<= 1)
            if (wv::ballot((warn & bit) != 0) != 0ull) w |= bit;
        if (lane == 0 && w) io.warn[env] |= w;
    }
    return (warn & WARN_DIVERGED) ? -2 : (bailed ? (bailed_down ? sub | ENV_STEP_WENT_DOWN : sub) : nsub);
}

template <int NVP, class TOPO, int FEAT = FEAT_ALL, int MAXR = MID_ROWS, int NW = 1, bool WALK = false, int WPS = NW, int INROWS = 0>
WV_GLOBAL void __launch_bounds__(WV_WAVE * NW) WV_OCC WV_WAVES_PER_SIMD(WPS) cassie_step_kernel(PhysIO io) {
    WV_SHARED EnvShared<NVP, LPack<TOPO, NVP>::count, MAXR> S;
    const int slot = wv::env_id();
    if constexpr (WALK) {
        wv::test_launch_hook(&S, sizeof S);
        const int count = wv::opaque(wv::shfl_i(wv::lane() == 0 ? wv::atomic_add(io.handover_count, 0) : 0, 0));
        for (int idx = slot; idx < count; idx += wv::grid_size()) {
            const int env = io.handover_list[io.env0 + idx];
            const long long t0 = io.cost ? wv::clock() : 0, t0w = io.cost_wall ? wv::wall_clock() : 0;
            env_step<NVP, TOPO, FEAT, MAXR, NW>(io, S, env, io.progress[env], io.nsub);
            if (io.cost && wv::lane() == 0 && (NW == 1 || wv::wave_id() == 0)) {
                io.cost[env] += (unsigned)((wv::clock() - t0) >> 6);
                if (io.cost_wall) io.cost_wall[env] += (unsigned)(wv::wall_clock() - t0w);
            }
            if constexpr (NW == 2) wv::block_barrier();
            else wv::sync();
        }
        if (wv::lane() == 0 && (NW == 1 || wv::wave_id() == 0) && wv::atomic_add(io.handover_count + 1, 1) == wv::grid_size() - 1) {
            io.handover_count[0] = 0; io.handover_count[1] = 0;
            if (io.handover_seen) *io.handover_seen = count;
        }
    } else {
    const int chunk = io.nchunk > 1 ? wv::env_id() / io.nenv : 0;
    const int eslot = slot - chunk * io.nenv;
    if (chunk >= (io.nchunk > 1 ? io.nchunk : 1)) return;
    wv::test_launch_hook(&S, sizeof S);
    const int env = io.order ? io.order[io.env0 + eslot] : io.env0 + eslot;
    int sub_start = io.resume ? io.progress[env] : 0, sub_end = io.nsub;
    if (io.nchunk > 1) {
        const int per = (io.nsub + io.nchunk - 1) / io.nchunk;
        sub_start = chunk * per;
        sub_end = sub_start + per < io.nsub ? sub_start + per : io.nsub;
    }
    if (sub_start >= io.nsub) return;
    if (chunk > 0) {
        if (!wv::wait_global<NW>(io.chunk_flag + env, io.chunk_seq, chunk)) {
            if (wv::lane() == 0) { wv::atomic_or(io.warn + env, WARN_CHUNK_PLACEMENT); if (io.chunk_fault) *io.chunk_fault = 1; }
        }
        if (io.progress[env] != sub_start) {
            if (sub_end < io.nsub) wv::publish_global<NW>(io.chunk_flag + env, io.chunk_seq, chunk + 1);
            return;
        }
    }
    const long long t0 = io.cost ? wv::clock() : 0, t0w = io.cost_wall ? wv::wall_clock() : 0;
    if constexpr (INROWS > 0) {
        static_assert(NW == 2 && INROWS > MAXR && INROWS <= MID_ROWS, "the in-place form: a two-wave fast instantiation with the 63-row code behind it");
        static_assert(sizeof(EnvShared<NVP, LPack<TOPO, NVP>::count, MAXR>) == sizeof(EnvShared<NVP, LPack<TOPO, NVP>::count, INROWS>), "both instantiations use the env's LDS block alike");
        auto &S2 = reinterpret_cast<EnvShared<NVP, LPack<TOPO, NVP>::count, INROWS> &>(S);
        PhysIO io2 = io;
        io2.has_next = io.inplace_has_next; io2.handover_out_list = io.inplace_out_list; io2.handover_out_count = io.inplace_out_count;
        io2.down_rows = io.inplace_stay_rows;
        const bool stay = io.inplace_stay_rows > 0;
        bool did = false;
        for (int s = sub_start;;) {
            int at = env_step<NVP, TOPO, FEAT, MAXR, NW>(io, S, env, s, sub_end);
            if (wv::lane() == 0 && wv::wave_id() == 0) S.cmd[5] = at;
            wv::drain_vmem(); wv::block_barrier();
            at = wv::opaque(S.cmd[5]);
            if (at < 0 || at >= sub_end) break;
            did = true;
            int at2 = env_step<NVP, TOPO, FEAT, INROWS, NW>(io2, S2, env, at, stay ? sub_end : at + 1);
            if (wv::lane() == 0 && wv::wave_id() == 0) S.cmd[5] = at2;
            wv::drain_vmem(); wv::block_barrier();
            at2 = wv::opaque(S.cmd[5]);
            if (at2 < 0) break;
            const bool down = (at2 & ENV_STEP_WENT_DOWN) != 0;
            at2 &= ENV_STEP_WENT_DOWN - 1;
            if (at2 >= sub_end) break;
            if (stay ? !down : at2 != at + 1) break;
            s = at2;
        }
        if (did && io.inplace_count && wv::lane() == 0 && wv::wave_id() == 0) wv::atomic_add(io.inplace_count, 1);
    } else env_step<NVP, TOPO, FEAT, MAXR, NW>(io, S, env, sub_start, sub_end);
    if (sub_end < io.nsub) wv::publish_global<NW>(io.chunk_flag + env, io.chunk_seq, chunk + 1);
    if (io.prof && wv::lane() == 0) io.prof[(size_t)env * NSTAMP + 40 + (NW == 2 ? wv::wave_id() : 0)] = wv::hw_id();
    if (io.prof && wv::lane() == 0 && (NW == 1 || wv::wave_id() == 0)) {
        io.prof[(size_t)env * NSTAMP + 42] = wv::clock(); io.prof[(size_t)env * NSTAMP + 43] = wv::wall_clock();
    }
    if (io.cost && wv::lane() == 0 && (NW == 1 || wv::wave_id() == 0)) {
        const unsigned c = (unsigned)((wv::clock() - t0) >> 6);
        io.cost[env] = io.resume || chunk > 0 ? io.cost[env] + c : c;
        if (io.cost_wall) { const unsigned cw = (unsigned)(wv::wall_clock() - t0w); io.cost_wall[env] = io.resume || chunk > 0 ? io.cost_wall[env] + cw : cw; }
    }
    }
}

}
#endif
```

cassie-mujoco-sim_amd/csrc/pk_types.h:

```cpp
#ifndef CASSIE_PK_TYPES_H
#define CASSIE_PK_TYPES_H

namespace ck {

constexpr int NB = CM_MAXBODY;
constexpr int NG = CM_MAXGEOM;
constexpr int NROW = 64;
constexpr int MID_ROWS = CM_MAXEFC_NARROW;
constexpr int WIDE_ROWS = CM_MAXEFC;
constexpr int FAST_ROWS = 31;
constexpr int FAST_ROWS_TRAY = 47;
constexpr int NSTAMP = 48;
#define CK_TRI(k, i) ((k) * ((k) + 1) / 2 + (i))
#define CK_STAMP(i) do { if (io.prof && lane == 0) io.prof[(size_t)env * NSTAMP + (i)] = wv::clock(); CK_FRESH(); } while (0)
#define CK_FRESH() do { lane = wv::fresh_lane(); b = lane; k_ = lane; isbody = b < nbody; isdof = k_ < nv; } while (0)

enum { WARN_CONTACT_FULL = 1, WARN_CONSTRAINT_FULL = 2, WARN_UNSUPPORTED_PAIR = 4, WARN_DIVERGED = 8,
       WARN_CHUNK_PLACEMENT = 16 ,
       WARN_TERRAIN_INDEX = 32   ,
       WARN_SCAN_TILTED = 64      };

#ifndef WV_OCC
#define WV_OCC
#endif
typedef const WV_CONST_AS cm_model_t *ModelPtr;
typedef const WV_CONST_AS cm_envparams_t *ParamPtr;

struct PhysIO {
    const cm_model_t *models;
    int model_stride;
    const cm_envparams_t *envparams;
    int nenv, nsub;
    int env0;
    int integrate;
    int sq, sqv, sv, su, ssd, sb;
    double *qpos, *qvel, *qacc_warmstart, *time;
    double *ctrl;
    const double *qfrc_applied, *xfrc_applied;
    double *qacc, *sensordata, *actuator_velocity;
    int *warn;
    int *info;
    double *xpos_out;
    double *xquat_out;
    double *body_cfrc;
    const float *hfield;
    size_t hfield_stride;
    const double *pd_ptarget, *pd_kp, *pd_kd;
    int drive_mode;
    cm_drive_state_t *drive_state;
    const double *drive_cmd;
    const double *pd_dtarget, *pd_torque;
    double *meas;
    cm_ext_t *ext;
    long long *prof;
    const int *order;
    unsigned *cost;
    unsigned *cost_wall;
    int all_outputs_every_substep;
    int *progress;
    int resume;
    int nchunk, chunk_seq;
    int *chunk_flag;
    volatile int *chunk_fault;
    int *handover_list, *handover_count;
    volatile int *handover_seen;
    int has_next;
    int *handover_out_list, *handover_out_count;
    int inplace_has_next;
    int *inplace_out_list, *inplace_out_count;
    int inplace_stay_rows;
    int down_rows;
    int *inplace_count;
    const int *hfield_index;
    int hfield_nterrain;
};

WV_DEVICE const float *terrain_grid(const float *hfield, size_t stride, const int *index, int nterrain, int env, bool *clamped) {
    *clamped = false;
    if (!hfield) return nullptr;
    if (!index) return hfield + (size_t)env * stride;
    const int want = index[env], last = nterrain - 1;
    const int t = want > last ? last : (want < 0 ? 0 : want);
    *clamped = t != want;
    return hfield + (size_t)(t < 0 ? 0 : t) * stride;
}

template <int NVP>
struct BodyTiles {
    double xpos[NB][3], xquat[NB][4], xmat[NB][9], xipos[NB][3];
    double xanchor[CM_MAXJNT][3], xaxis[CM_MAXJNT][3];
    double cinert[NB][10], crb[NB][10];
    double cvel[NB][6], cfrc[NB][6];
    double cdof_dot[NVP][6], buf[NVP][6];
    double geom_xpos[NG][3], geom_xmat[NG][9];
};
template <int NVP, int MAXR, bool SEPARATE> struct TilesAndY {
    static constexpr int YP = NVP + 2;
    union { BodyTiles<NVP> s; double Yr[MAXR + 1][YP]; };
};
template <int NVP, int MAXR> struct TilesAndY<NVP, MAXR, true> {
    static constexpr int YP = NVP + 2;
    BodyTiles<NVP> s;
    double Yr[MAXR + 1][YP];
    double rowt[MAXR + 1][4];
    double vx[2][NVP];
    double sums[8];
    int turn[4];
    double stepv[2][NROW];
    double chg[NROW];
};
template <int NVP, int NL = NVP * (NVP + 1) / 2, int MAXR = MID_ROWS>
struct EnvShared {
    static constexpr int YP = NVP + 2;
    static constexpr bool WIDE = MAXR > MID_ROWS;
    static constexpr int MAXC = WIDE ? CM_MAXCON : CM_MAXCON_NARROW;
    TilesAndY<NVP, MAXR, WIDE> x;
    double Lp[NL], LHp[NL];
    double accel[2][28];
    double dinv[NVP], rsd[NVP], dinvH[NVP];
    double cdof[NVP][6];
    double com[NB][3];
    double qpos[CM_MAXQ], qvel[NVP], qacc_ws[NVP], qacc[NVP], ctrl[CM_MAXU];
    double qfrc_smooth[NVP];
    double sens[CM_MAXSENSORDATA], actvel[CM_MAXU];
    int drv_x[CM_NUM_DRIVES][CM_DRIVE_FILTER_NB];
    double drv_jx[CM_NUM_JOINTS][CM_JOINT_FILTER_NB], drv_jy[CM_NUM_JOINTS][CM_JOINT_FILTER_NA];
    double drv_delay[CM_NUM_DRIVES][CM_TORQUE_DELAY_CYCLES];
    double drv_pos[CM_NUM_DRIVES], drv_vel[CM_NUM_DRIVES];
    double drv_c[CM_NUM_DRIVES][10], drv_jc[CM_NUM_JOINTS][2];
    int drv_msg[2];
    double c_dist[MAXC], c_pos[MAXC][3], c_frame[MAXC][9], c_fri[MAXC][3];
    double c_solref[MAXC][2], c_solimp[MAXC][5], c_margin[MAXC];
    int c_dim[MAXC], c_g1[MAXC], c_g2[MAXC], c_pair[MAXC];
    int c_root[MAXC][2];
    unsigned long long c_dofmask[MAXC][2];
    double c_tran[MAXC];
    int cmd[6];
};

}
#endif
```

Before: 27.56 million.

## Re-derive launch args and model pointers from kernarg segment at stage boundaries

Result: slower. 27.26 million (-1.1%).

```diff
diff --git a/cassie-mujoco-sim_amd/csrc/env_step_collision.inc b/cassie-mujoco-sim_amd/csrc/env_step_collision.inc
--- a/cassie-mujoco-sim_amd/csrc/env_step_collision.inc
+++ b/cassie-mujoco-sim_amd/csrc/env_step_collision.inc
@@ -41,7 +41,7 @@
             }
             if (wv::ballot(nearby) != 0ull) npass = m->npair_simple;
         }
-        CK_STAMP(21);
+        CK_STAGE(21);
         constexpr int HF_REC = 1 + 10 * CM_HF_MAXC;
         static_assert(CM_MAXHFPAIR * HF_REC <= NB * 12 + NVP * 12, "the height-field result table must fit the cvel + cfrc + cdof_dot + buf tiles");
         static_assert(offsetof(decltype(S.x.s), buf) - offsetof(decltype(S.x.s), cvel) == sizeof(double) * (NB * 12 + NVP * 6), "those four tiles are contiguous");
@@ -52,9 +52,9 @@
         int ncon_prism = 0;
         if constexpr ((FEAT & FEAT_HFIELD) != 0) if (hf_prism) {
             static_assert(CM_MAXHFPAIR * HP_REC + 64 * 2 * CM_HP_MAXS / 8 <= NB * 12 + NVP * 12, "the per-pair records of the prism pass and its task table (a byte per task) fit the idle velocity tiles");
-            CK_STAMP(44);
+            CK_STAGE(44);
             ncon_prism = hfield_prism_wave(S, m, env_hfield, lane, hfres, MAXC);
-            CK_STAMP(46);
+            CK_STAGE(46);
         }
         if constexpr ((FEAT & FEAT_HFIELD) != 0) if (hf_on && !hf_prism) {
             const bool dense = (m->flags & CM_FLAG_HFDENSE) != 0;
@@ -86,9 +86,9 @@
                     double e[3] = {p2[0] + t * axis[0], p2[1] + t * axis[1], p2[2] + t * axis[2]};
                     static_assert(offsetof(SH_T, c_tran) + sizeof(S.c_tran) - offsetof(SH_T, c_dist) >= (size_t)HF_WORK_BYTES,
                                   "the contact tables hold the work area of hfield_spheres_wave");
-                    CK_STAMP(44);
+                    CK_STAGE(44);
                     has = hfield_spheres_wave(rcs, m, env_hfield, p1, m1, mine, e, s20, margin, lane, &S.c_dist[0]) != 0;
-                    CK_STAMP(45);
+                    CK_STAGE(45);
                 }
                 const int lead = lane - k;
                 double dk[CM_HF_SLOTS_DENSE];
@@ -135,7 +135,7 @@
                 }
             }
             wv::sync();
-            CK_STAMP(46);
+            CK_STAGE(46);
         }
         if constexpr (!request_early) request_pair(lane, pc);
         if constexpr ((FEAT & FEAT_HFIELD) != 0) ncon = ncon_prism;
@@ -170,7 +170,7 @@
                 const double rb1 = pc.rb1, rb2 = pc.rb2;
                 const double s10 = pc.s10, s11 = pc.s11, s20 = pc.s20, s21 = pc.s21, s22 = pc.s22;
                 double dif[3] = {p2[0] - p1[0], p2[1] - p1[1], p2[2] - p1[2]};
-                CK_STAMP(31);
+                CK_STAGE(31);
                 bool cull = false;
                 if (rb1 > 0 && rb2 > 0) {
                     double bound = rb1 + rb2 + margin;
@@ -216,7 +216,7 @@
                     }
                 }
             }
-            CK_STAMP(32);
+            CK_STAGE(32);
             if (p0 + WV_WAVE < npass) request_pair(p + WV_WAVE, pc);
             const unsigned long long m1b = wv::ballot(n >= 1), m2b = wv::ballot(n >= 2);
             const unsigned long long below = (lane == 0) ? 0ull : (~0ull >> (64 - lane));
@@ -239,7 +239,7 @@
             if (n >= 2 && slot + 1 < MAXC) write_raw_contact(S, slot + 1, p, rc1);
             ncon += wv::popc64(m1b) + wv::popc64(m2b) + more;
         }
-        CK_STAMP(22);
+        CK_STAGE(22);
         if constexpr (!request_early) request_behind_collision(lane);
         if constexpr ((FEAT & FEAT_WAVEPAIRS) != 0) for (int p = m->npair_simple; p < m->npair; ++p) {
             const int g1 = m->pair_geom1[p], g2 = m->pair_geom2[p], tt = m->pair_type[p];
@@ -303,7 +303,7 @@
             lob = wv::ballot(lo); hib = wv::ballot(hi);
         }
         if constexpr (MAXR < WIDE_ROWS) {
-            const bool may_go_down = io.down_rows > 0 && sub > sub_start;
+            const bool may_go_down = io->down_rows > 0 && sub > sub_start;
             if (can_hand_over || may_go_down) {
                 const int neq = m->neq;
                 const bool eact = lane < neq && m->eq_active[lane < neq ? lane : 0] != 0;
@@ -311,7 +311,7 @@
                 const int nfrictionless = wv::popc64(wv::ballot(lane < ncon && S.c_dim[lane < MAXC ? lane : 0] == 1));
                 const int need = 3 * wv::popc64(wv::ballot(eact)) + wv::popc64(lob) + wv::popc64(hib) + 4 * ncon - 3 * nfrictionless;
                 const bool up = can_hand_over && (need > capr || (ncon_found > capc && MAXC < m->maxcon));
-                const bool down = !up && may_go_down && need <= io.down_rows;
+                const bool down = !up && may_go_down && need <= io->down_rows;
                 if (up || down) {
                     bailed = true; bailed_down = down;
                     if constexpr (NW == 2) { if (lane == 0) S.cmd[0] = 1; wv::publish(&S.cmd[4], sub + 1); }
@@ -320,9 +320,9 @@
             }
         }
         if (ncon_found > capc) warn |= WARN_CONTACT_FULL;
-        if constexpr (NW == 1) if (io.drive_mode) {
-            if (io.integrate) drive_level_io(io, S, m, env, lane, lastsub);
+        if constexpr (NW == 1) if (io->drive_mode) {
+            if (io->integrate) drive_level_io(io, S, m, env, lane, lastsub);
             wv::sync();
         }
-        if constexpr (NW == 2) { CK_STAMP(33); wv::publish(&S.cmd[4], sub + 1); wv::wait_for(&S.cmd[3], sub + 1); }
-        CK_STAMP(5);
+        if constexpr (NW == 2) { CK_STAGE(33); wv::publish(&S.cmd[4], sub + 1); wv::wait_for(&S.cmd[3], sub + 1); }
+        CK_STAGE(5);
diff --git a/cassie-mujoco-sim_amd/csrc/env_step_rows.inc b/cassie-mujoco-sim_amd/csrc/env_step_rows.inc
--- a/cassie-mujoco-sim_amd/csrc/env_step_rows.inc
+++ b/cassie-mujoco-sim_amd/csrc/env_step_rows.inc
@@ -2,8 +2,8 @@
         int rtype = -1, rid = 0, rsub = 0;
         int nefc = 0, nefc_before_contacts = 0;
         double rpos = 0, rmargin = 0, rR = 1.0, rK = 0, rB = 0, rimp = 1.0;
-        const bool need_imu = lastsub || io.all_outputs_every_substep || (io.drive_mode && sub + 2 == nsub);
-        const bool need_pos = lastsub || io.drive_mode || io.all_outputs_every_substep;
+        const bool need_imu = lastsub || io->all_outputs_every_substep || (io->drive_mode && sub + 2 == nsub);
+        const bool need_pos = lastsub || io->drive_mode || io->all_outputs_every_substep;
         const bool issens = lane < m->nsensor && need_pos;
         const int ls = issens ? lane : 0;
         SensorConsts sens_c;
@@ -60,7 +60,7 @@
             nefc += nrow;
         }
 
-        CK_STAMP(25);
+        CK_STAGE(25);
         double u3[3] = {0, 0, 0}, wp[3] = {0, 0, 0}, wm[3] = {0, 0, 0};
         unsigned long long maskp = 0, maskm = 0;
         int limdof = -1;
@@ -129,7 +129,7 @@
             solref0 = S.c_solref[c][0]; solref1 = S.c_solref[c][1];
             for (int i = 0; i < 5; ++i) solimp[i] = S.c_solimp[c][i];
         }
-        CK_STAMP(26);
+        CK_STAGE(26);
         if (rtype >= 0) {
             rimp = impedance(solimp, imp_pos, rmargin);
             rR = fmax(CM_MINVAL, (1 - rimp) * rdiag / rimp);
@@ -145,7 +145,7 @@
                 rB = -solref1 / fmax(CM_MINVAL, dmax);
             }
         }
-        CK_STAMP(27);
+        CK_STAGE(27);
         if constexpr (NW == 1) sens_c = request_sensor_consts(m, ls);
 #pragma unroll
         for (int k0 = 0; k0 < NVP; k0 += 4) {
@@ -186,8 +186,8 @@
                 rt[0] = rR; rt[1] = rtype >= 0 ? -rB * jvel - rK * rimp * (rpos - rmargin) : 0.0; rt[2] = jws;
                 rt[3] = rtype < 0 ? -1.0 : (rtype == CM_CNSTR_EQUALITY ? 0.0 : 1.0);
             }
-            if (io.ext && pass == 0 && rtype == CM_CNSTR_EQUALITY && r_ < CM_MAXEQROW) {
-                cm_ext_t *ex = io.ext + env;
+            if (io->ext && pass == 0 && rtype == CM_CNSTR_EQUALITY && r_ < CM_MAXEQROW) {
+                cm_ext_t *ex = io->ext + env;
                 ex->eq_pos[r_] = rpos; ex->eq_id[r_] = rid;
 #pragma unroll
                 for (int k = 0; k < NVP; ++k) if (k < nv) ex->eq_J[r_][k] = ycol[k];
@@ -195,10 +195,10 @@
         }
         }
         const int sb = NW == 1 ? sens_c.sb : 0;
-        CK_STAMP(28);
+        CK_STAGE(28);
         if constexpr (NW == 2) {
             if constexpr (WIDE) { if (lane == 0) S.x.turn[0] = nefc; }
-            CK_STAMP(34); wv::block_barrier();
+            CK_STAGE(34); wv::block_barrier();
             if (lastcol) {
 #pragma unroll
                 for (int k = 0; k < NVP; ++k) ycol[k] = (TOPO::is_static ? k < TOPO::nv : k < nv) ? S.qfrc_smooth[k] : 0.0;
@@ -208,13 +208,13 @@
 
         int aslot = -1;
         if constexpr (NW == 1) aslot = sensors_before_solve(io, S, m, env, issens, ls, sens_c, need_imu, lastsub);
-        CK_STAMP(29);
-        if (io.xpos_out && isbody && lastsub) {
-            for (int i = 0; i < 3; ++i) io.xpos_out[((size_t)env * io.sb + b) * 3 + i] = S.x.s.xpos[b][i];
-            if (io.xquat_out) for (int i = 0; i < 4; ++i) io.xquat_out[((size_t)env * io.sb + b) * 4 + i] = S.x.s.xquat[b][i];
-        }
-        if (io.ext) {
-            cm_ext_t *ex = io.ext + env;
+        CK_STAGE(29);
+        if (io->xpos_out && isbody && lastsub) {
+            for (int i = 0; i < 3; ++i) io->xpos_out[((size_t)env * io->sb + b) * 3 + i] = S.x.s.xpos[b][i];
+            if (io->xquat_out) for (int i = 0; i < 4; ++i) io->xquat_out[((size_t)env * io->sb + b) * 4 + i] = S.x.s.xquat[b][i];
+        }
+        if (io->ext) {
+            cm_ext_t *ex = io->ext + env;
             if (isbody) for (int i = 0; i < 6; ++i) ex->cvel[b][i] = S.x.s.cvel[b][i];
             if (isbody) for (int i = 0; i < 3; ++i) { ex->subtree_com[b][i] = S.com[broot > 0 ? broot : 0][i]; ex->xipos[b][i] = S.x.s.xipos[b][i]; }
             if (lane < m->nsite) {
@@ -244,8 +244,8 @@
             }
         }
         int caddr = -1;
-        const bool want_cfrc = io.body_cfrc && (sub == nsub - 1 || !io.integrate);
-        if (io.ext || want_cfrc) {
+        const bool want_cfrc = io->body_cfrc && (sub == nsub - 1 || !io->integrate);
+        if (io->ext || want_cfrc) {
             int acc = nefc_before_contacts;
             for (int c = 0; c < ncon; ++c) {
                 const int dim = S.c_dim[c];
@@ -257,4 +257,4 @@
             }
         }
         wv::sync();
-        CK_STAMP(8);
+        CK_STAGE(8);
diff --git a/cassie-mujoco-sim_amd/csrc/env_step_solve.inc b/cassie-mujoco-sim_amd/csrc/env_step_solve.inc
--- a/cassie-mujoco-sim_amd/csrc/env_step_solve.inc
+++ b/cassie-mujoco-sim_amd/csrc/env_step_solve.inc
@@ -1,7 +1,7 @@
         if constexpr (WIDE) {
             int iters = 0, nguarded = 0;
             const double f = wide_solve<NVP, TOPO>(S, m, P, 0, nefc, sub, iters, nguarded);
-            CK_STAMP(11);
+            CK_STAGE(11);
 
             static_assert(sizeof(S.c_solimp) >= (2 * NROW + 4) * sizeof(double), "the row forces are handed over through the contacts' solimp slots");
             double *const fbuf = &S.c_solimp[0][0];
@@ -9,9 +9,9 @@
             if (lane == 0) { fbuf[2 * NROW] = (double)ncon; fbuf[2 * NROW + 1] = (double)nefc; fbuf[2 * NROW + 2] = (double)iters; fbuf[2 * NROW + 3] = (double)nguarded; }
             wv::block_barrier();
 #ifdef CK_WIDE_PROFILE
-            if (io.prof && lane < 12) io.prof[(size_t)env * NSTAMP + (lane < 6 ? 16 + lane : 22 + lane)] = (long long)S.x.stepv[lane / 6][lane % 6];
+            if (io->prof && lane < 12) io->prof[(size_t)env * NSTAMP + (lane < 6 ? 16 + lane : 22 + lane)] = (long long)S.x.stepv[lane / 6][lane % 6];
 #endif
-            if (io.ext || want_cfrc) {
+            if (io->ext || want_cfrc) {
                 const int a0 = caddr >= 0 ? caddr : 0;
                 double fn = 0, ft1 = 0, ft2 = 0;
                 if (lane < ncon && caddr >= 0) {
@@ -19,8 +19,8 @@
                     if (S.c_dim[lane] == 1) fn = f0;
                     else { const double f1 = fbuf[a0 + 1], f2 = fbuf[a0 + 2], f3 = fbuf[a0 + 3], mu = S.c_fri[lane][0]; fn = f0 + f1 + f2 + f3; ft1 = mu * (f0 - f1); ft2 = mu * (f2 - f3); }
                 }
-                if (io.ext) {
-                    cm_ext_t *ex = io.ext + env;
+                if (io->ext) {
+                    cm_ext_t *ex = io->ext + env;
                     if (lane < ncon) { ex->con_force[lane][0] = fn; ex->con_force[lane][1] = ft1; ex->con_force[lane][2] = ft2; }
                     if (lane == 0) { ex->ncon = ncon; ex->nefc = nefc; ex->solver_iter = iters; }
                 }
@@ -39,15 +39,15 @@
                             const double sg = (b2 == b ? 1.0 : 0.0) - (b1 == b ? 1.0 : 0.0);
                             for (int j = 0; j < 3; ++j) acc[j] += sg * S.c_pos[c][j];
                         }
-                        for (int j = 0; j < 3; ++j) io.body_cfrc[((size_t)env * io.sb + b) * 3 + j] = acc[j];
+                        for (int j = 0; j < 3; ++j) io->body_cfrc[((size_t)env * io->sb + b) * 3 + j] = acc[j];
                     }
                     wv::sync();
                 }
             }
             wv::block_barrier();
-            CK_STAMP(37);
+            CK_STAGE(37);
             if (wv::opaque(S.cmd[0])) { warn |= WARN_DIVERGED; break; }
-            if (!io.integrate) break;
+            if (!io->integrate) break;
             time += h;
             continue;
         }
@@ -92,7 +92,7 @@
         }
         wv::sync();
         if constexpr (NW == 2) wv::publish(&S.cmd[2], sub + 1);
-        CK_STAMP(9);
+        CK_STAGE(9);
 
         double arow[MAXR];
         double diag_yy = 0;
@@ -247,7 +247,7 @@
             rb = acc - raref;
         }
         }
-        CK_STAMP(10);
+        CK_STAGE(10);
 
         const bool isrow = rtype >= 0;
         const bool clampf = isrow && rtype != CM_CNSTR_EQUALITY;
@@ -293,7 +293,7 @@
                 if (cost > 0) f = 0;
                 else if (isrow) res = rb + af;
             }
-        CK_STAMP(30);
+        CK_STAGE(30);
             const double scale = 1.0 / (P->meaninertia * (nv > 1 ? nv : 1));
             const double halfAii = 0.5 * Aii;
             const double flo = clampf ? 0.0 : -1e300;
@@ -346,8 +346,8 @@
             }
         }
         if constexpr (NW == 2 && CK_PRIO_W0_PGS != CK_PRIO_W0) wv::set_priority<CK_PRIO_W0>();
-        CK_STAMP(11);
-        if (io.ext || want_cfrc) {
+        CK_STAGE(11);
+        if (io->ext || want_cfrc) {
             const int a0 = caddr >= 0 ? caddr : 0;
             const double f0 = wv::shfl(f, a0), f1 = wv::shfl(f, (a0 + 1) & 63), f2 = wv::shfl(f, (a0 + 2) & 63), f3 = wv::shfl(f, (a0 + 3) & 63);
             double fn = 0, ft1 = 0, ft2 = 0;
@@ -355,8 +355,8 @@
                 if (S.c_dim[lane] == 1) fn = f0;
                 else { const double mu = S.c_fri[lane][0]; fn = f0 + f1 + f2 + f3; ft1 = mu * (f0 - f1); ft2 = mu * (f2 - f3); }
             }
-            if (io.ext) {
-                cm_ext_t *ex = io.ext + env;
+            if (io->ext) {
+                cm_ext_t *ex = io->ext + env;
                 if (lane < ncon) { ex->con_force[lane][0] = fn; ex->con_force[lane][1] = ft1; ex->con_force[lane][2] = ft2; }
                 if (lane == 0) { ex->ncon = ncon; ex->nefc = nefc; ex->solver_iter = iters; }
             }
@@ -375,7 +375,7 @@
                         const double sg = (b2 == b ? 1.0 : 0.0) - (b1 == b ? 1.0 : 0.0);
                         for (int j = 0; j < 3; ++j) acc[j] += sg * S.c_pos[c][j];
                     }
-                    for (int j = 0; j < 3; ++j) io.body_cfrc[((size_t)env * io.sb + b) * 3 + j] = acc[j];
+                    for (int j = 0; j < 3; ++j) io->body_cfrc[((size_t)env * io->sb + b) * 3 + j] = acc[j];
                 }
                 wv::sync();
             }
@@ -388,9 +388,9 @@
             if (lane == 0) { fbuf[64] = (double)ncon; fbuf[65] = (double)nefc; fbuf[66] = (double)iters; fbuf[67] = (double)nguarded; }
             wv::block_barrier();
             wv::block_barrier();
-            CK_STAMP(37);
+            CK_STAGE(37);
             if (wv::opaque(S.cmd[0])) { warn |= WARN_DIVERGED; break; }
-            if (!io.integrate) break;
+            if (!io->integrate) break;
             time += h;
             continue;
         }
@@ -424,11 +424,11 @@
         }
         if (isdof) S.qacc[k_] = qacc;
         wv::sync();
-        CK_STAMP(12);
+        CK_STAGE(12);
 
         outputs_after_qacc(io, S, m, env, lane, isdof, k_, nu, qacc, aslot, sb, need_imu, lastsub, pf_agear * S.qvel[pf_adof], ncon, nefc, iters, nguarded);
-        if (!io.integrate) break;
-        CK_STAMP(13);
+        if (!io->integrate) break;
+        CK_STAGE(13);
 
         {
             double lcol[NVP], lrowh[NVP];
@@ -437,5 +437,5 @@
             euler_step<NVP, TOPO>(S, m, lane, isdof, k_, nv, njnt, h, qacc, lcol, lrowh, dih, pf_kdamp, pf_ejt, pf_eqa, pf_eda);
         }
         time += h;
-        CK_STAMP(14);
+        CK_STAGE(14);
     }
diff --git a/cassie-mujoco-sim_amd/csrc/env_step_wave1.inc b/cassie-mujoco-sim_amd/csrc/env_step_wave1.inc
--- a/cassie-mujoco-sim_amd/csrc/env_step_wave1.inc
+++ b/cassie-mujoco-sim_amd/csrc/env_step_wave1.inc
@@ -6,11 +6,11 @@
                 double iner[3], imat[9];
                 for (int i = 0; i < 3; ++i) iner[i] = P->body_inertia[pb][i];
                 for (int i = 0; i < 9; ++i) imat[i] = m->body_imat[pb][i];
-                CK_STAMP(35);
+                CK_STAGE(35);
                 wv::block_barrier();
                 if (wv::opaque(S.cmd[0])) return -1;
                 wv::set_priority<(FEAT & FEAT_HFIELD) != 0 ? CK_PRIO_W1_FJ_HFIELD : CK_PRIO_W1_FJ>();
-                CK_STAMP(36);
+                CK_STAGE(36);
                 double ximat[9] = {1, 0, 0, 0, 1, 0, 0, 0, 1};
                 if (isbody && b > 0) {
                     double xm[9];
@@ -21,7 +21,7 @@
                 double col[NVP], colh[NVP];
                 mass_matrix_columns<NVP, TOPO, FEAT, NW>(io, S, m, env, ids, mass, iner, ximat, col, colh);
                 wv::publish(&S.cmd[3], sub1 + 1);
-                CK_STAMP(38);
+                CK_STAGE(38);
                 factor_pair_by_height<NVP, TOPO, 0>(m, P, h, S, col, colh, lane);
                 constexpr bool park_colh = NVP > 32;
                 if constexpr (park_colh) {
@@ -37,11 +37,11 @@
                 }
                 wv::wait_for(&S.cmd[4], sub1 + 1);
                 if (wv::opaque(S.cmd[0])) return -1;
-                if (io.drive_mode) {
-                    if (io.integrate) drive_level_io(io, S, m, env, lane, sub1 == nsub - 1);
+                if (io->drive_mode) {
+                    if (io->integrate) drive_level_io(io, S, m, env, lane, sub1 == nsub - 1);
                     wv::sync();
                 }
-                CK_STAMP(4);
+                CK_STAGE(4);
                 {
                     const int kd = isdof ? k_ : 0;
                     const double kdamp = P->dof_damping[kd], kstiff = PS->dof_stiffness[kd], kref = PS->dof_springref[kd];
@@ -50,16 +50,16 @@
                     wv::wait_for(&S.cmd[1], sub1 + 1);
                     bias_forces_and_qfrc_smooth<NVP, (NVP > 32)>(io, S, m, env, ids, kdamp, kstiff, kref, kgear, klo, khi, kq, ka);
                 }
-                const bool lastsub1 = sub1 == nsub - 1 || !io.integrate;
-                const bool need_imu1 = lastsub1 || io.all_outputs_every_substep || (io.drive_mode && sub1 + 2 == nsub);
-                const bool issens1 = lane < m->nsensor && (lastsub1 || io.drive_mode || io.all_outputs_every_substep);
+                const bool lastsub1 = sub1 == nsub - 1 || !io->integrate;
+                const bool need_imu1 = lastsub1 || io->all_outputs_every_substep || (io->drive_mode && sub1 + 2 == nsub);
+                const bool issens1 = lane < m->nsensor && (lastsub1 || io->drive_mode || io->all_outputs_every_substep);
                 const int ls1 = issens1 ? lane : 0;
                 const SensorConsts sens_c1 = request_sensor_consts(m, ls1);
                 const int aslot1 = sensors_before_solve(io, S, m, env, issens1, ls1, sens_c1, need_imu1, lastsub1);
-                CK_STAMP(47);
+                CK_STAGE(47);
                 wv::block_barrier();
                 wv::set_priority<CK_PRIO_W1_JP>();
-                CK_STAMP(39);
+                CK_STAGE(39);
                 if constexpr (WIDE) {
                     int it1 = 0, ng1 = 0;
                     const double f1 = wide_solve<NVP, TOPO>(S, m, P, 1, wv::opaque(S.x.turn[0]), sub1, it1, ng1);
@@ -147,18 +147,18 @@
                     if (isdof) S.qacc[k_] = qacc;
                     const double av = pf_agear * S.qvel[pf_adof];
                     wv::sync();
-                    CK_STAMP(12);
-                    if (io.integrate) {
+                    CK_STAGE(12);
+                    if (io->integrate) {
                         if constexpr (!stage_h_early) stage_factor_h<NVP, TOPO>(S, k_, isdof, nv, lcol, lrowh);
                         euler_step<NVP, TOPO>(S, m, lane, isdof, k_, nv, njnt, h, qacc, lcol, lrowh, dih, pf_kdamp, pf_ejt, pf_eqa, pf_eda);
                     }
-                    CK_STAMP(13);
+                    CK_STAGE(13);
                     wv::block_barrier();
                     wv::set_priority<CK_PRIO_W1_EF>();
                     outputs_after_qacc(io, S, m, env, lane, isdof, k_, nu, qacc, aslot, sb, need_imu, lastsub, av, ncon, nefc, iters, nguarded);
-                    CK_STAMP(14);
+                    CK_STAGE(14);
                 }
-                if (!io.integrate || ++sub1 >= nsub) return -1;
+                if (!io->integrate || ++sub1 >= nsub) return -1;
             }
         }
     }
diff --git a/cassie-mujoco-sim_amd/csrc/physics_kernel.h b/cassie-mujoco-sim_amd/csrc/physics_kernel.h
--- a/cassie-mujoco-sim_amd/csrc/physics_kernel.h
+++ b/cassie-mujoco-sim_amd/csrc/physics_kernel.h
@@ -19,8 +19,10 @@
 
 constexpr int ENV_STEP_WENT_DOWN = 1 << 20;
 
-template <int NVP, class TOPO, int FEAT, int MAXR, int NW>
-WV_DEVICE int env_step(const PhysIO &io, EnvShared<NVP, LPack<TOPO, NVP>::count, MAXR> &S, int env, int sub_start, int nsub) {
+template <int NVP, class TOPO, int FEAT, int MAXR, int NW, bool KARG = true>
+WV_DEVICE int env_step(const PhysIO &io_launch, EnvShared<NVP, LPack<TOPO, NVP>::count, MAXR> &S, int env, int sub_start, int nsub) {
+    constexpr bool fresh_args = KARG && NW == 2 && TOPO::is_static && TOPO::nv == NVP;
+    LaunchArgs<fresh_args> io(io_launch);
     typedef LPack<TOPO, NVP> LP;
     static_assert(NW == 1 || NW == 2, "one or two wavefronts per env");
     static_assert(NW == 1 || TOPO::is_static, "the two-wave form exists for the compile-time topologies");
@@ -33,35 +35,36 @@
     constexpr int MAXC = SH_T::MAXC;
     constexpr bool WIDE = SH_T::WIDE;
     static_assert(!WIDE || (NW == 2 && MAXR == WIDE_ROWS), "the 127-row instantiation spreads its solve over the two wavefronts of an env");
-    const ModelPtr m_launch = (ModelPtr)(io.models + (size_t)env * io.model_stride);
+    const ModelPtr m_launch = (ModelPtr)(io->models + (size_t)env * io->model_stride);
     ModelPtr m = m_launch;
-    const ParamPtr P = io.envparams ? (ParamPtr)(io.envparams + (size_t)env) : (ParamPtr)&m_launch->params;
-    const ParamPtr PG = m_launch->env_geom ? P : (ParamPtr)&m_launch->params, PS = m_launch->env_springs ? P : (ParamPtr)&m_launch->params;
+    ParamPtr P = io->envparams ? (ParamPtr)(io->envparams + (size_t)env) : (ParamPtr)&m_launch->params;
+    ParamPtr PG = m_launch->env_geom ? P : (ParamPtr)&m_launch->params, PS = m_launch->env_springs ? P : (ParamPtr)&m_launch->params;
     int lane = wv::lane();
-    const int nq = m->nq, nv = m->nv, nu = m->nu, nbody = m->nbody, njnt = m->njnt;
+    const int nv = (TOPO::is_static && TOPO::nv == NVP) ? TOPO::nv : m->nv;
+    const int nq = m->nq, nu = m->nu, nbody = m->nbody, njnt = m->njnt;
     const int capr = m->maxefc < MAXR ? m->maxefc : MAXR, capc = m->maxcon < MAXC ? m->maxcon : MAXC;
-    const bool can_hand_over = MAXR < WIDE_ROWS && io.has_next != 0 && io.progress != nullptr && (MAXR < m->maxefc || MAXC < m->maxcon);
+    const bool can_hand_over = MAXR < WIDE_ROWS && io->has_next != 0 && io->progress != nullptr && (MAXR < m->maxefc || MAXC < m->maxcon);
     const double h = m->timestep;
     int warn = 0;
 
     if (NW == 1 || wid == 0) {
     if (lane == 0) { S.cmd[0] = 0; S.cmd[1] = 0; S.cmd[2] = 0; S.cmd[3] = 0; S.cmd[4] = 0; }
     if constexpr (WIDE) { if (lane == 0) { S.x.turn[0] = 0; S.x.turn[1] = 0; S.x.turn[2] = 0; S.x.turn[3] = 0; } }
-    if (lane < nq) S.qpos[lane] = io.qpos[(size_t)env * io.sq + lane];
+    if (lane < nq) S.qpos[lane] = io->qpos[(size_t)env * io->sq + lane];
     if (lane < nv) {
-        S.qvel[lane] = io.qvel[(size_t)env * io.sqv + lane];
-        S.qacc_ws[lane] = io.qacc_warmstart[(size_t)env * io.sv + lane];
-    }
-    if (lane < nu) S.ctrl[lane] = io.ctrl[(size_t)env * io.su + lane];
+        S.qvel[lane] = io->qvel[(size_t)env * io->sqv + lane];
+        S.qacc_ws[lane] = io->qacc_warmstart[(size_t)env * io->sv + lane];
+    }
+    if (lane < nu) S.ctrl[lane] = io->ctrl[(size_t)env * io->su + lane];
     if (lane < NB && !wv::test_skip_com_init()) { S.com[lane][0] = 0.0; S.com[lane][1] = 0.0; S.com[lane][2] = 0.0; }
-    if (io.drive_mode) {
-        if (lane < m->nsensordata) S.sens[lane] = io.sensordata[(size_t)env * io.ssd + lane];
-        if (lane < nu) S.actvel[lane] = io.actuator_velocity[(size_t)env * io.su + lane];
+    if (io->drive_mode) {
+        if (lane < m->nsensordata) S.sens[lane] = io->sensordata[(size_t)env * io->ssd + lane];
+        if (lane < nu) S.actvel[lane] = io->actuator_velocity[(size_t)env * io->su + lane];
         drive_state_load(io, S, env, lane);
         drive_consts_load(io, S, m, env, lane);
     }
     }
-    double time = io.time[env];
+    double time = io->time[env];
 
     int b = lane;
     bool isbody = b < nbody;
@@ -95,15 +98,15 @@
     const float *env_hfield = nullptr;
     if constexpr ((FEAT & FEAT_HFIELD) != 0) {
         bool clamped;
-        env_hfield = terrain_grid(io.hfield, io.hfield_stride, io.hfield_index, io.hfield_nterrain, env, &clamped);
-        if (clamped && lane == 0 && wid == 0) wv::atomic_or(io.warn + env, WARN_TERRAIN_INDEX);
+        env_hfield = terrain_grid(io->hfield, io->hfield_stride, io->hfield_index, io->hfield_nterrain, env, &clamped);
+        if (clamped && lane == 0 && wid == 0) wv::atomic_or(io->warn + env, WARN_TERRAIN_INDEX);
     }
 
     bool bailed = false, bailed_down = false;
     int sub = sub_start;
     for (; sub < nsub; ++sub) {
-        const bool lastsub = sub == nsub - 1 || !io.integrate;
-        const bool need_quat = lastsub || io.ext != nullptr || io.all_outputs_every_substep || (io.drive_mode && sub + 2 == nsub);
+        const bool lastsub = sub == nsub - 1 || !io->integrate;
+        const bool need_quat = lastsub || io->ext != nullptr || io->all_outputs_every_substep || (io->drive_mode && sub + 2 == nsub);
         {
             bool badv = false;
             if (lane < nq) { double v = S.qpos[lane]; badv |= !(v == v) || fabs(v) > 1e10; }
@@ -114,20 +117,20 @@
                 break;
             }
         }
-        if (io.drive_mode) {
-        } else if (io.pd_ptarget) {
+        if (io->drive_mode) {
+        } else if (io->pd_ptarget) {
             if (lane < nu) {
-                const size_t o = (size_t)env * io.su + lane;
+                const size_t o = (size_t)env * io->su + lane;
                 const double ratio = m->act_gear[lane], tmax = m->act_ctrlrange[lane][1];
                 const double q = S.qpos[m->act_qposadr[lane]], qd = S.qvel[m->act_dofid[lane]];
-                const double tau = io.pd_kp[o] * (io.pd_ptarget[o] - q) - io.pd_kd[o] * qd;
+                const double tau = io->pd_kp[o] * (io->pd_ptarget[o] - q) - io->pd_kd[o] * qd;
                 const double wmax = m->act_maxrpm[lane] * (2.0 * 3.14159265358979323846 / 60.0);
                 const double tlim = clampd(2 * tmax * (1 - fabs(ratio * qd) / wmax), 0.0, tmax);
                 S.ctrl[lane] = copysign(fmin(fabs(tau / ratio), tlim), tau);
             }
             wv::sync();
         }
-        CK_STAMP(0);
+        CK_STAGE(0);
         if constexpr (NW == 2 && prio_kin != CK_PRIO_W0) wv::set_priority<prio_kin>();
 
         double Rl[9] = {1, 0, 0, 0, 1, 0, 0, 0, 1}, pl[3] = {0, 0, 0}, qlq[4] = {1, 0, 0, 0};
@@ -243,7 +246,7 @@
                 }
             }
         }
-        CK_STAMP(16);
+        CK_STAGE(16);
         const int pf_b = isbody ? b : 0, pf_g = lane < m->ngeom ? lane : -1, pf_gs = pf_g >= 0 ? pf_g : 0;
         const int pf_jpb = lane < njnt ? m->jnt_parentbody[lane] : -1, pf_gb = m->geom_bodyid[pf_gs];
         const double pf_mass = P->body_mass[pf_b];
@@ -322,7 +325,7 @@
         }
         if constexpr (NW == 2) wv::block_barrier();
         if constexpr (NW == 2 && prio_kin != CK_PRIO_W0) wv::set_priority<CK_PRIO_W0>();
-        CK_STAMP(1);
+        CK_STAGE(1);
 
         if (pf_g >= 0) {
             const int g = pf_g, gb = pf_gb;
@@ -336,7 +339,7 @@
         }
         if constexpr (NW == 2) wv::sync();
 
-        CK_STAMP(17);
+        CK_STAGE(17);
         double col[NVP], colh[NVP];
         if constexpr (NW == 1) mass_matrix_columns<NVP, TOPO, FEAT, NW>(io, S, m, env, ids, pf_mass, pf_iner, ximat, col, colh);
 
@@ -354,7 +357,7 @@
                 }
             }
         }
-        if constexpr (NW == 1) CK_STAMP(4);
+        if constexpr (NW == 1) CK_STAGE(4);
 
 #include "env_step_collision.inc"
 
@@ -406,7 +409,7 @@
                 for (int t = 0; t < 6; ++t) term[t] = 0;
             }
             wv::sync();
-            CK_STAMP(23);
+            CK_STAGE(23);
             chain_sums(term);
             for (int t = 0; t < 6; ++t) mycacc[t] = blast >= 0 ? S.x.s.buf[blast >= 0 ? blast : 0][t] : 0.0;
             mycacc[3] -= m->gravity[0]; mycacc[4] -= m->gravity[1]; mycacc[5] -= m->gravity[2];
@@ -427,7 +430,7 @@
             for (int i = 0; i < 6; ++i) S.x.s.cfrc[lane][i] = f6[i];
         }
         wv::sync();
-        CK_STAMP(24);
+        CK_STAGE(24);
         if constexpr (NW == 2) {
             wv::publish(&S.cmd[1], sub + 1);
         } else bias_forces_and_qfrc_smooth<NVP>(io, S, m, env, ids, kdamp, kstiff, kref, kgear, klo, khi, kq, ka);
@@ -438,35 +441,36 @@
 
 #include "env_step_solve.inc"
 
-    if (io.progress && lane == 0 && (!io.resume || bailed)) {
-        io.progress[env] = bailed ? sub : nsub;
-        if (bailed && !bailed_down && io.handover_out_list) io.handover_out_list[io.env0 + wv::atomic_add(io.handover_out_count, 1)] = env;
-    }
-    if (io.integrate && io.drive_mode) {
+    CK_FRESH_ARGS();
+    if (io->progress && lane == 0 && (!io->resume || bailed)) {
+        io->progress[env] = bailed ? sub : nsub;
+        if (bailed && !bailed_down && io->handover_out_list) io->handover_out_list[io->env0 + wv::atomic_add(io->handover_out_count, 1)] = env;
+    }
+    if (io->integrate && io->drive_mode) {
         drive_state_store(io, S, env, lane);
-        if (lane < nu) io.ctrl[(size_t)env * io.su + lane] = S.ctrl[lane];
+        if (lane < nu) io->ctrl[(size_t)env * io->su + lane] = S.ctrl[lane];
         if (bailed) {
-            if (lane < m->nsensordata) io.sensordata[(size_t)env * io.ssd + lane] = S.sens[lane];
-            if (lane < nu) io.actuator_velocity[(size_t)env * io.su + lane] = S.actvel[lane];
+            if (lane < m->nsensordata) io->sensordata[(size_t)env * io->ssd + lane] = S.sens[lane];
+            if (lane < nu) io->actuator_velocity[(size_t)env * io->su + lane] = S.actvel[lane];
             if (lane < CM_NUM_DRIVES) {
-                double *meas = io.meas + (size_t)env * CM_MEAS_DIM;
+                double *meas = io->meas + (size_t)env * CM_MEAS_DIM;
                 meas[CM_MEAS_DRIVE_POS + lane] = S.drv_pos[lane]; meas[CM_MEAS_DRIVE_VEL + lane] = S.drv_vel[lane];
             }
         }
     }
-    if (io.integrate) {
-        if (lane < nq) io.qpos[(size_t)env * io.sq + lane] = S.qpos[lane];
+    if (io->integrate) {
+        if (lane < nq) io->qpos[(size_t)env * io->sq + lane] = S.qpos[lane];
         if (lane < nv) {
-            io.qvel[(size_t)env * io.sqv + lane] = S.qvel[lane];
-            io.qacc_warmstart[(size_t)env * io.sv + lane] = S.qacc_ws[lane];
-        }
-        if (lane == 0) io.time[env] = time;
+            io->qvel[(size_t)env * io->sqv + lane] = S.qvel[lane];
+            io->qacc_warmstart[(size_t)env * io->sv + lane] = S.qacc_ws[lane];
+        }
+        if (lane == 0) io->time[env] = time;
     }
     {
         int w = 0;
         for (int bit = 1; bit <= 8; bit <<= 1)
             if (wv::ballot((warn & bit) != 0) != 0ull) w |= bit;
-        if (lane == 0 && w) io.warn[env] |= w;
+        if (lane == 0 && w) io->warn[env] |= w;
     }
     return (warn & WARN_DIVERGED) ? -2 : (bailed ? (bailed_down ? sub | ENV_STEP_WENT_DOWN : sub) : nsub);
 }
@@ -532,7 +536,7 @@
             at = wv::opaque(S.cmd[5]);
             if (at < 0 || at >= sub_end) break;
             did = true;
-            int at2 = env_step<NVP, TOPO, FEAT, INROWS, NW>(io2, S2, env, at, stay ? sub_end : at + 1);
+            int at2 = env_step<NVP, TOPO, FEAT, INROWS, NW, false>(io2, S2, env, at, stay ? sub_end : at + 1);
             if (wv::lane() == 0 && wv::wave_id() == 0) S.cmd[5] = at2;
             wv::drain_vmem(); wv::block_barrier();
             at2 = wv::opaque(S.cmd[5]);
diff --git a/cassie-mujoco-sim_amd/csrc/pk_types.h b/cassie-mujoco-sim_amd/csrc/pk_types.h
--- a/cassie-mujoco-sim_amd/csrc/pk_types.h
+++ b/cassie-mujoco-sim_amd/csrc/pk_types.h
@@ -13,6 +13,8 @@
 constexpr int NSTAMP = 48;
 #define CK_TRI(k, i) ((k) * ((k) + 1) / 2 + (i))
 #define CK_STAMP(i) do { if (io.prof && lane == 0) io.prof[(size_t)env * NSTAMP + (i)] = wv::clock(); CK_FRESH(); } while (0)
+#define CK_STAGE(i) do { if (io->prof && lane == 0) io->prof[(size_t)env * NSTAMP + (i)] = wv::clock(); CK_FRESH(); CK_FRESH_ARGS(); } while (0)
+#define CK_FRESH_ARGS() do { if constexpr (fresh_args) { io.refresh(); m = wv::opaque_ptr(m); P = wv::opaque_ptr(P); PG = wv::opaque_ptr(PG); PS = wv::opaque_ptr(PS); } } while (0)
 #define CK_FRESH() do { lane = wv::fresh_lane(); b = lane; k_ = lane; isbody = b < nbody; isdof = k_ < nv; } while (0)
 
 enum { WARN_CONTACT_FULL = 1, WARN_CONSTRAINT_FULL = 2, WARN_UNSUPPORTED_PAIR = 4, WARN_DIVERGED = 8,
@@ -73,6 +75,18 @@
     int *inplace_count;
     const int *hfield_index;
     int hfield_nterrain;
+};
+
+template <bool KARG> struct LaunchArgs {
+    const PhysIO *p;
+    WV_DEVICE explicit LaunchArgs(const PhysIO &io) : p(&io) { refresh(); }
+    WV_DEVICE void refresh() {
+#ifndef CK_EMULATED
+        if constexpr (KARG) p = (const PhysIO *)wv::opaque_ptr((const WV_CONST_AS PhysIO *)__builtin_amdgcn_kernarg_segment_ptr());
+#endif
+    }
+    WV_DEVICE const PhysIO *operator->() const { return p; }
+    WV_DEVICE operator const PhysIO &() const { return *p; }
 };
 
 WV_DEVICE const float *terrain_grid(const float *hfield, size_t stride, const int *index, int nterrain, int env, bool *clamped) {
```
